# OliBomby/CM3P

Measured on AMD Instinct MI355X. Metric: contrastive training steps/sec (global beatmap-metadata pairs/sec), higher is better.
Workload: dtype bf16; 1 GPU; c2: default CM3P config, beatmap seq=4096, metadata seq=256, batch 32/GPU; global_batch=32, beatmap_seq=4096, metadata_seq=256, parallelism=dp1, weights=random init (reference init rules), fp32 master / bf16 GEMM operands

## Files before the change

cm3p_amd/_lib.py:

```python
from __future__ import annotations

import ctypes
import os
from ctypes import c_float, c_int, c_int64, c_uint64, c_void_p

import torch

F32, BF16 = 0, 1
ADD_A_BF16 = 16
POOL_PACKED = 2
GEMM_F32_TILED = 2
EPI_BF16, EPI_F32, EPI_F32_RESID, EPI_F32_BIAS, EPI_BF16_RESID = 0, 1, 2, 5, 7
EPI_BF16_GEGLU_FWD, EPI_BF16_GEGLU_BWD = 9, 10
ABI_VERSION = 20

_HERE = os.path.dirname(os.path.abspath(__file__))
LIB_PATH = os.environ.get("CM3P_HIP_LIB") or os.path.join(_HERE, "csrc", "libcm3p_hip.so")

_P, _I, _L, _F, _U64 = c_void_p, c_int, c_int64, c_float, c_uint64
_RETURNS_INT64 = {"cm3p_attn_bwd_fused_workspace_bytes", "cm3p_token_order_workspace_ints"}

SIGNATURES = {
    "cm3p_abi_version": [],
    "cm3p_layernorm_fwd": [_P, _I, _P, _P, _P, _P, _P, _L, _I, _F, _P],
    "cm3p_layernorm_bwd_blocks": [_L],
    "cm3p_layernorm_bwd": [_P, _I, _P, _I, _P, _P, _P, _P, _I, _P, _P, _P, _P, _L, _I, _P],
    "cm3p_embed_ln_fwd": [_P, _P, _I, _P, _P, _I, _P, _P, _P, _P, _P, _L, _I, _F, _L, _P],
    "cm3p_embed_ln_bwd": [_P, _I, _P, _P, _I, _P, _P, _I, _P, _P, _P, _P, _P, _P, _P, _L, _I, _L, _L, _P],
    "cm3p_embed_ln_bwd_sorted_chunk": [],
    "cm3p_embed_ln_bwd_sorted": [_P, _I, _P, _P, _P, _P, _I, _P, _P, _I, _P, _P, _P, _P, _P, _P, _P, _P, _P, _L, _I, _L, _L, _P],
    "cm3p_token_order_workspace_ints": [_L, _L],
    "cm3p_token_order": [_P, _L, _L, _P, _P, _P, _P],
    "cm3p_audio_slots": [_P, _L, _L, _P, _P, _P],
    "cm3p_gemm_bf16": [_P, _P, _P, _P, _L, _L, _L, _L, _L, _L, _I, _I, _I, _I, _P, _P],
    "cm3p_qkv_gemm_rope": [_P, _P, _P, _L, _L, _L, _P, _P, _I, _I, _I, _F, _P],
    "cm3p_gemm_wgrad_splits": [_L, _L, _L],
    "cm3p_gemm_route": [_L, _L, _L, _L, _L, _I, _I, _I, _I, _I, _I],
    "cm3p_gemm8p_set_grid": [_I],
    "cm3p_gemm8p_get_grid": [],
    "cm3p_build_ablation_flags": [],
    "cm3p_debug_set_dma_audit": [_P],
    "cm3p_cast_f32_bf16": [_P, _P, _L, _P],
    "cm3p_cast_f32_bf16_t": [_P, _P, _P, _L, _L, _P],
    "cm3p_cast_f32_bf16_t_multi": [_P, _I, _L, _P],
    "cm3p_add_f32": [_P, _P, _I, _P, _P, _L, _P],
    "cm3p_rope_table": [_P, _L, _P, _I, _P, _P, _P],
    "cm3p_rope_apply": [_P, _P, _P, _I, _I, _I, _L, _I, _P],
    "cm3p_attn_fwd": [_P, _P, _P, _P, _I, _I, _I, _I, _F, _I, _P],
    "cm3p_attn_fwd_impl": [_I, _I, _I, _I],
    "cm3p_attn_probs": [_P, _P, _P, _P, _I, _I, _I, _I, _F, _I, _P],
    "cm3p_attn_generic_supported": [_I],
    "cm3p_attn_fwd_generic": [_P, _P, _P, _P, _I, _I, _I, _I, _I, _F, _P],
    "cm3p_attn_bwd_generic": [_P, _P, _P, _P, _P, _P, _P, _I, _I, _I, _I, _I, _F, _P],
    "cm3p_attn_fwd_generic_dropout": [_P, _P, _P, _P, _I, _I, _I, _I, _I, _F, _I, _I, _U64, _P],
    "cm3p_attn_bwd_generic_dropout": [_P, _P, _P, _P, _P, _P, _P, _I, _I, _I, _I, _I, _F, _I, _I, _U64, _P],
    "cm3p_rope_apply_generic": [_P, _P, _P, _I, _I, _I, _I, _L, _I, _P],
    "cm3p_attn_bwd": [_P, _P, _P, _P, _P, _P, _P, _I, _I, _I, _I, _F, _P, _P, _L, _I, _I, _P],
    "cm3p_geglu_fwd": [_P, _P, _L, _I, _P],
    "cm3p_gemm_geglu": [_P, _P, _P, _L, _L, _L, _P],
    "cm3p_geglu_bwd": [_P, _P, _P, _L, _I, _P],
    "cm3p_dropout_f32": [_P, _P, _P, _P, _L, _I, _I, _P, _I, _I, _I, _I, _U64, _P],
    "cm3p_attn_fwd_dropout": [_P, _P, _P, _P, _I, _I, _I, _I, _F, _I, _I, _I, _U64, _P],
    "cm3p_attn_bwd_dropout": [_P, _P, _P, _P, _P, _P, _P, _I, _I, _I, _I, _F, _P, _P, _L, _I, _I, _I, _I, _U64, _P],
    "cm3p_attn_fwd_dropout_varlen": [_P, _P, _P, _P, _I, _I, _L, _I, _I, _F, _I, _I, _I, _U64, _P],
    "cm3p_attn_bwd_dropout_varlen": [_P, _P, _P, _P, _P, _P, _P, _I, _I, _L, _I, _I, _F, _P, _P, _I, _I, _I, _I, _U64, _P],
    "cm3p_geglu_fwd_dropout": [_P, _P, _L, _I, _I, _P, _I, _I, _I, _U64, _P],
    "cm3p_geglu_bwd_dropout": [_P, _P, _P, _L, _I, _I, _P, _I, _I, _I, _U64, _P],
    "cm3p_dropout_keep": [_P, _I, _I, _I, _I, _I, _I, _U64, _P],
    "cm3p_philox4x32_10_host": [_P, _P, _P, _L],
    "cm3p_gelu_fwd": [_P, _P, _L, _P],
    "cm3p_gelu_bwd": [_P, _P, _P, _L, _P],
    "cm3p_im2col_k3": [_P, _I, _P, _I, _I, _I, _I, _I, _P],
    "cm3p_col2im_k3": [_P, _P, _I, _I, _I, _I, _I, _P],
    "cm3p_bias_gelu_fwd": [_P, _P, _P, _P, _L, _I, _P],
    "cm3p_bias_gelu_bwd_blocks": [_L],
    "cm3p_bias_gelu_bwd": [_P, _I, _P, _P, _P, _P, _P, _L, _I, _P],
    "cm3p_pool_chunks": [_I],
    "cm3p_pool_fwd": [_P, _I, _P, _P, _P, _P, _I, _I, _I, _I, _P],
    "cm3p_pool_bwd": [_P, _P, _P, _P, _I, _I, _I, _I, _I, _P],
    "cm3p_gemm_f32": [_P, _P, _P, _I, _I, _I, _L, _L, _L, _L, _L, _F, _I, _P],
    "cm3p_l2norm_fwd": [_P, _P, _P, _I, _I, _P],
    "cm3p_l2norm_bwd": [_P, _P, _P, _P, _I, _I, _P],
    "cm3p_cross_entropy": [_P, _I, _I, _L, _L, _P, _P, _F, _P, _P, _P],
    "cm3p_cross_entropy_masked": [_P, _L, _I, _L, _P, _L, _F, _P, _P, _P, _P],
    "cm3p_inv_valid_count": [_P, _L, _L, _P, _P],
    "cm3p_ce_masked_stats": [_P, _L, _I, _L, _P, _L, _P, _P, _P],
    "cm3p_ce_masked_dlogits_blocks": [_L],
    "cm3p_ce_masked_dlogits_bf16": [_P, _L, _I, _L, _P, _L, _P, _P, _P, _P, _P, _P, _P],
    "cm3p_add_bias_f32": [_P, _P, _L, _I, _P],
    "cm3p_colsum_blocks": [_L],
    "cm3p_colsum_f32": [_P, _P, _P, _L, _I, _P],
    "cm3p_first_zero_index": [_P, _I, _I, _P, _P],
    "cm3p_scale_exp": [_P, _P, _P, _L, _P],
    "cm3p_scale_by": [_P, _P, _P, _L, _P],
    "cm3p_dot_f32": [_P, _P, _P, _L, _P],
    "cm3p_sum_f32": [_P, _P, _L, _F, _I, _P],
# ... 158 lines not shown
```

cm3p_amd/csrc/attention_bwd_fused.hip:

```cpp
#include <stdlib.h>

#include <type_traits>

#include "attn_common.h"

namespace {

#ifndef CM3P_FABL
#define CM3P_FABL 0
#endif

#ifndef CM3P_FTRACE
#define CM3P_FTRACE 0
#endif
#if CM3P_FTRACE
__device__ unsigned long long* g_bwdf_trace = nullptr;
#endif

constexpr int kFStage = 16384 + 512;
constexpr int kFSlots = 3;
constexpr int kFKimg = kFSlots * kFStage;
constexpr int kFdS = kFKimg + 32768;
constexpr int kFZ = kFdS + 2 * 32768;
constexpr int kFLds = kFZ + 4 * 2560;
constexpr int kFUnroll = 6;
constexpr int kFPadTiles = 12;

__host__ __device__ inline int64_t fused_stat_floats(int B, int S, int nh) { return (int64_t)B * nh * ((S + 63) / 64 + kFPadTiles) * 128; }
__host__ __device__ inline int fused_slab_rows(int S) { return ((S + 63) / 64) * 64 + 64; }
__host__ __device__ inline int fused_slabs(int S, int G = 2) { return ((S + 255) / 256 + G - 1) / G; }

__device__ __forceinline__ bf16x8 gload_frag8(const uint16_t* p) { return *reinterpret_cast<const bf16x8*>(p); }

__device__ __forceinline__ void mfma_av0(f32x16& d, const bf16x8& a, const bf16x8& b) {
    asm volatile("v_mfma_f32_32x32x16_bf16 %0, %1, %2, 0" : "=&v"(d) : "a"(a), "v"(b));
}
__device__ __forceinline__ void mfma_ava(f32x16& d, const bf16x8& a, const bf16x8& b) {
    asm volatile("v_mfma_f32_32x32x16_bf16 %0, %1, %2, %0" : "+v"(d) : "a"(a), "v"(b));
}
__device__ __forceinline__ void mfma_vva(f32x16& d, const bf16x8& a, const bf16x8& b) {
    asm volatile("v_mfma_f32_32x32x16_bf16 %0, %1, %2, %0" : "+v"(d) : "v"(a), "v"(b));
}

__device__ __forceinline__ void lds_barrier() {
    asm volatile("s_waitcnt lgkmcnt(0)" ::: "memory");
    __builtin_amdgcn_s_barrier();
    asm volatile("" ::: "memory");
}

template <bool PRE>
__device__ __forceinline__ void exp2c_pair(f32x16& s, int i, float cm) {
    if constexpr ((CM3P_FABL & 64) != 0) return;
    s[i] = __builtin_amdgcn_fmed3f(__builtin_amdgcn_exp2f(PRE ? s[i] : s[i] * cm), 0.f, 1.f);
    s[i + 1] = __builtin_amdgcn_fmed3f(__builtin_amdgcn_exp2f(PRE ? s[i + 1] : s[i + 1] * cm), 0.f, 1.f);
}

__global__ __launch_bounds__(256) void attn_bwd_prep_kernel(const uint16_t* __restrict__ o_rows, const uint16_t* __restrict__ d_o,
                                                            const float* __restrict__ lse, float* __restrict__ stat_ws, int Smax, int nh,
                                                            float lse_mul, VarLen vl) {
    const int t = blockIdx.x, head = blockIdx.y, b = blockIdx.z, tid = threadIdx.x;
    const SeqView sv(vl, b, head, Smax, nh);
    const int S = sv.S;
    const int row = t * 64 + (tid >> 2), part = tid & 3;
    const int64_t ldo = (int64_t)nh * 64;
    float acc = 0.f;
    if (row < S) {
        const uint16_t* po = o_rows + (sv.row0 + row) * ldo + head * 64 + part * 16;
        const uint16_t* pg = d_o + (sv.row0 + row) * ldo + head * 64 + part * 16;
#pragma unroll
        for (int h = 0; h < 2; ++h) {
            const bf16x8 a = gload_frag8(po + 8 * h), g = gload_frag8(pg + 8 * h);
#pragma unroll
            for (int j = 0; j < 8; ++j) acc += (float)a[j] * (float)g[j];
        }
    }
    acc += __shfl_xor(acc, 1, 64);
    acc += __shfl_xor(acc, 2, 64);
    if (part == 0) {
        float* st = stat_ws + (((int64_t)b * nh + head) * gridDim.x + t) * 128;
        const bool ok = row < S;
        st[tid >> 2] = ok ? lse[sv.stat0 + row] * lse_mul : kNegInf;
        st[64 + (tid >> 2)] = ok ? -acc : 0.f;
    }
}

__device__ __forceinline__ void dq_reduce_tile(const uint16_t* __restrict__ dq_part, uint16_t* __restrict__ dqkv, int t, int head, int b,
                                               int tid, const SeqView& sv, int Smax, int nh, float scale,
                                               const float* __restrict__ rope_cos, const float* __restrict__ rope_sin,
                                               int64_t pos_batch_stride, int G) {
    const int S = sv.S;
    const int row = t * 64 + (tid >> 2), j = tid & 3;
    if (row >= S) return;
    const int nkb = fused_slabs(Smax, G), nkb_b = fused_slabs(S, G);
    const int64_t slab = (int64_t)fused_slab_rows(Smax) * 64;
    const uint16_t* p = dq_part + ((int64_t)b * nh + head) * nkb * slab + (int64_t)row * 64 + 8 * j;
    float lo[8], hi[8];
#pragma unroll
    for (int i = 0; i < 8; ++i) lo[i] = hi[i] = 0.f;
    constexpr int kBatch = 8;
    for (int kb0 = 0; kb0 < nkb_b; kb0 += kBatch) {
        uint4 a[kBatch], c[kBatch];
#pragma unroll
        for (int u = 0; u < kBatch; ++u) {
            const int kb = min(kb0 + u, nkb_b - 1);
            a[u] = gload16<(CM3P_NT & 8) != 0>(p + kb * slab);
            c[u] = gload16<(CM3P_NT & 8) != 0>(p + kb * slab + 32);
        }
#pragma unroll
        for (int u = 0; u < kBatch; ++u) {
            if (kb0 + u < nkb_b) {
                lo[0] += bf16lo(a[u].x), lo[1] += bf16hi(a[u].x), lo[2] += bf16lo(a[u].y), lo[3] += bf16hi(a[u].y);
                lo[4] += bf16lo(a[u].z), lo[5] += bf16hi(a[u].z), lo[6] += bf16lo(a[u].w), lo[7] += bf16hi(a[u].w);
                hi[0] += bf16lo(c[u].x), hi[1] += bf16hi(c[u].x), hi[2] += bf16lo(c[u].y), hi[3] += bf16hi(c[u].y);
                hi[4] += bf16lo(c[u].z), hi[5] += bf16hi(c[u].z), hi[6] += bf16lo(c[u].w), hi[7] += bf16hi(c[u].w);
            }
        }
    }
    if (rope_cos) {
        const int64_t prow = sv.pos0(b, pos_batch_stride) + row;
#pragma unroll
        for (int h = 0; h < 2; ++h) {
            f32x4 lo4 = {lo[4 * h], lo[4 * h + 1], lo[4 * h + 2], lo[4 * h + 3]};
            f32x4 hi4 = {hi[4 * h], hi[4 * h + 1], hi[4 * h + 2], hi[4 * h + 3]};
            rope_rotate4<true>(lo4, hi4, rope_cos + prow * 32, rope_sin + prow * 32, 8 * j + 4 * h);
#pragma unroll
            for (int r = 0; r < 4; ++r) {
                lo[4 * h + r] = lo4[r];
                hi[4 * h + r] = hi4[r];
            }
        }
    }
    uint16_t* drow = dqkv + (sv.row0 + row) * ((int64_t)3 * nh * 64) + head * 64 + 8 * j;
    gstore16<(CM3P_NT & 8) != 0>(drow, uint4{pack_bf16x2(lo[0] * scale, lo[1] * scale), pack_bf16x2(lo[2] * scale, lo[3] * scale),
                                             pack_bf16x2(lo[4] * scale, lo[5] * scale), pack_bf16x2(lo[6] * scale, lo[7] * scale)});
    gstore16<(CM3P_NT & 8) != 0>(drow + 32, uint4{pack_bf16x2(hi[0] * scale, hi[1] * scale), pack_bf16x2(hi[2] * scale, hi[3] * scale),
                                                  pack_bf16x2(hi[4] * scale, hi[5] * scale), pack_bf16x2(hi[6] * scale, hi[7] * scale)});
}

__global__ __launch_bounds__(256) void attn_bwd_dq_reduce_kernel(const uint16_t* __restrict__ dq_part, uint16_t* __restrict__ dqkv, int Smax,
                                                                 int nh, float scale, const float* __restrict__ rope_cos,
                                                                 const float* __restrict__ rope_sin, int64_t pos_batch_stride, VarLen vl, int G) {
    const int head = blockIdx.y, b = blockIdx.z;
    const SeqView sv(vl, b, head, Smax, nh);
    dq_reduce_tile(dq_part, dqkv, blockIdx.x, head, b, threadIdx.x, sv, Smax, nh, scale, rope_cos, rope_sin, pos_batch_stride, G);
}

template <bool PRE, bool ADD>
__global__ __launch_bounds__(256, 1) void attn_bwd_fused_kernel(const uint16_t* __restrict__ qkv, const uint16_t* __restrict__ d_o,
                                                                const float* __restrict__ stat_ws, uint16_t* __restrict__ dq_part,
                                                                uint16_t* __restrict__ dqkv, const uint8_t* __restrict__ kmask, int Smax,
                                                                int nh, float scale, const float* __restrict__ rope_cos,
                                                                const float* __restrict__ rope_sin, int64_t pos_batch_stride, VarLen vl, int G,
                                                                int phase) {
    extern __shared__ __attribute__((aligned(16))) char smem[];
    const int tid = threadIdx.x, lane = tid & 63, hh = lane >> 5;
    const int wid = __builtin_amdgcn_readfirstlane(tid >> 6);
    const int nkb = (Smax + 255) / 256, NT = (Smax + 63) / 64;
    const int nblk = (nkb - phase + G - 1) / G;
    int kblk, head, b;
    decode_block(nblk, nh, kblk, head, b);
    const int slab_idx = kblk;
    kblk = G * kblk + phase;
    const int K0 = kblk * 256;
    const SeqView sv(vl, b, head, Smax, nh);
    const int S = sv.S;
// ... 419 lines not shown
            loadG_one(smem, sp, db, 0);
            loadG_one(smem, sp, db, 1);
        }
    mfma_vc(sA, Qf[0], kf[0][0], isv);
    mfma_vc(dpA, Gf[0], vf[0][0], idv);
#pragma unroll
    for (int s4 = 1; s4 < 4; ++s4) {
        mfma_va(sA, Qf[s4], kf[0][s4]);
        mfma_va(dpA, Gf[s4], vf[0][s4]);
    }
#pragma unroll
    for (int i = 0; i < 16; ++i) dq[i] = 0.f;
    load_dq_operand(dqB0, 1, 8);
    asm volatile("s_nop 15\n\ts_nop 15" ::: "memory");
    CM3P_SB();

#if CM3P_FTRACE
    const unsigned long long ft0 = __builtin_amdgcn_s_memtime();
#endif
    for (int t = 0; t < n_tiles + 2; t += kFUnroll) {
        tile(std::integral_constant<int, 0>{}, I0{}, t);
        tile(std::integral_constant<int, 1>{}, I1{}, t + 1);
        tile(std::integral_constant<int, 2>{}, I0{}, t + 2);
        tile(std::integral_constant<int, 0>{}, I1{}, t + 3);
        tile(std::integral_constant<int, 1>{}, I0{}, t + 4);
        tile(std::integral_constant<int, 2>{}, I1{}, t + 5);
    }
    asm volatile("s_waitcnt vmcnt(0)" ::: "memory");
#if CM3P_FTRACE
    if (g_bwdf_trace && lane == 0) {
        unsigned long long* o = g_bwdf_trace + (size_t)blockIdx.x * 16 + wid * 4;
        o[0] = ft_acc[0];
        o[1] = ft_acc[1];
        o[2] = __builtin_amdgcn_s_memtime() - ft0;
        o[3] = (unsigned long long)(n_tiles + 2 + kFUnroll - 1) / kFUnroll * kFUnroll;
    }
#endif


#pragma unroll
    for (int kb = 0; kb < 2; ++kb) {
        const int krow = k0 + 32 * kb + l31;
        if (krow < S) {
            const bool ok = kmask ? kmask[sv.row0 + krow] != 0 : true;
            const float ks = ok ? (PRE ? 0.69314718055994531f : scale) : 0.f, vs = ok ? 1.f : 0.f;
            uint16_t* dkrow = dqkv + (sv.row0 + krow) * ld + nh * 64 + head * 64;
            uint16_t* dvrow = dkrow + nh * 64;
            if (!ok) {
#pragma unroll
                for (int db = 0; db < 2; ++db)
#pragma unroll
                    for (int i = 0; i < 16; ++i) dk[db][kb][i] = dv[db][kb][i] = 0.f;
            }
            if (rope_cos) {
                const int64_t prow = sv.pos0(b, pos_batch_stride) + krow;
#pragma unroll
                for (int g = 0; g < 4; ++g) {
                    f32x4 lo4 = {dk[0][kb][4 * g], dk[0][kb][4 * g + 1], dk[0][kb][4 * g + 2], dk[0][kb][4 * g + 3]};
                    f32x4 hi4 = {dk[1][kb][4 * g], dk[1][kb][4 * g + 1], dk[1][kb][4 * g + 2], dk[1][kb][4 * g + 3]};
                    rope_rotate4<true>(lo4, hi4, rope_cos + prow * 32, rope_sin + prow * 32, 8 * g + 4 * hh);
#pragma unroll
                    for (int r = 0; r < 4; ++r) {
                        dk[0][kb][4 * g + r] = lo4[r];
                        dk[1][kb][4 * g + r] = hi4[r];
                    }
                }
            }
#pragma unroll
            for (int db = 0; db < 2; ++db)
#pragma unroll
                for (int g = 0; g < 4; ++g) {
                    const int d = 32 * db + 8 * g + 4 * hh;
                    *reinterpret_cast<uint2*>(dkrow + d) = uint2{pack_bf16x2(dk[db][kb][4 * g] * ks, dk[db][kb][4 * g + 1] * ks),
                                                                 pack_bf16x2(dk[db][kb][4 * g + 2] * ks, dk[db][kb][4 * g + 3] * ks)};
                    *reinterpret_cast<uint2*>(dvrow + d) = uint2{pack_bf16x2(dv[db][kb][4 * g] * vs, dv[db][kb][4 * g + 1] * vs),
                                                                 pack_bf16x2(dv[db][kb][4 * g + 2] * vs, dv[db][kb][4 * g + 3] * vs)};
                }
        }
    }
}

}

extern "C" {

int cm3p_attn_bwd_fused_slab_group(int S) {
    const char* e = getenv("CM3P_FUSED_SLAB_GROUP");
    if (e && (e[0] == '2' || e[0] == '4') && e[1] == '\0') return e[0] - '0';
    return (S + 255) / 256 >= 24 ? 4 : 2;
}

int64_t cm3p_attn_bwd_fused_workspace_bytes(int B, int S, int nh) {
    if (B <= 0 || S <= 0 || nh <= 0) return 0;
    const int64_t stats = (fused_stat_floats(B, S, nh) * 4 + 255) / 256 * 256;
    return stats + (int64_t)B * nh * fused_slabs(S) * fused_slab_rows(S) * 128;
}

int cm3p_attn_bwd_fused(const void* qkv, const void* out, const void* dout, const float* lse, void* dqkv, const uint8_t* key_mask,
                        const int* cu_seqlens, int B, int S, int64_t total, int nh, float scale, const float* cos_tab,
                        const float* sin_tab, int64_t pos_batch_stride, int stages, int q_prescaled, void* workspace,
                        int64_t workspace_bytes, void* stream) {
    CM3P_REQUIRE((cos_tab == nullptr) == (sin_tab == nullptr));
    CM3P_REQUIRE(stages >= 1 && stages <= 255);
    CM3P_REQUIRE(qkv && out && dout && lse && dqkv && workspace && B > 0 && S > 0 && nh > 0 && scale > 0.f);
    CM3P_REQUIRE(cm3p_aligned16(qkv) && cm3p_aligned16(out) && cm3p_aligned16(dout) && cm3p_aligned16(dqkv) && cm3p_aligned16(workspace));
    if (cu_seqlens) CM3P_REQUIRE(total > 0 && key_mask == nullptr && pos_batch_stride == 0);
    else CM3P_REQUIRE(pos_batch_stride == 0 || pos_batch_stride == S);
    CM3P_REQUIRE(workspace_bytes >= cm3p_attn_bwd_fused_workspace_bytes(B, S, nh));
    CM3P_REQUIRE((int64_t)S * 3 * nh * 128 < (int64_t)1 << 31);
    hipStream_t s = static_cast<hipStream_t>(stream);
    const VarLen vl{cu_seqlens, cu_seqlens ? total : 0};
    float* stat_ws = static_cast<float*>(workspace);
    uint16_t* dq_part = reinterpret_cast<uint16_t*>(static_cast<char*>(workspace) + (fused_stat_floats(B, S, nh) * 4 + 255) / 256 * 256);
    const int NT = (S + 63) / 64;
    const bool pre = q_prescaled != 0;
    const int G = cm3p_attn_bwd_fused_slab_group(S);
    CM3P_REQUIRE((stages & (7 * CM3P_ATTN_BWD_FUSED_MAIN_ADD1) & ~(((1 << (G - 1)) - 1) * CM3P_ATTN_BWD_FUSED_MAIN_ADD1)) == 0);
    if (stages & CM3P_ATTN_BWD_FUSED_PREP) {
        const float lse_mul = pre ? -kLog2e : -1.0f / scale;
        attn_bwd_prep_kernel<<<dim3(NT + kFPadTiles, nh, B), 256, 0, s>>>((const uint16_t*)out, (const uint16_t*)dout, lse, stat_ws, S, nh,
                                                                          lse_mul, vl);
        if (hipGetLastError() != hipSuccess) return CM3P_ERR_LAUNCH;
    }
    const bool run_even = stages & (CM3P_ATTN_BWD_FUSED_MAIN | CM3P_ATTN_BWD_FUSED_MAIN_EVEN);
    const bool run_odd = stages & (CM3P_ATTN_BWD_FUSED_MAIN | CM3P_ATTN_BWD_FUSED_MAIN_ODD);
    if (run_even || run_odd || (stages & (7 * CM3P_ATTN_BWD_FUSED_MAIN_ADD1))) {
        static Cm3pDevOnce once;
        const int rc_once = once.run([] {
            return cm3p_set_max_lds({reinterpret_cast<const void*>(&attn_bwd_fused_kernel<true, false>), reinterpret_cast<const void*>(&attn_bwd_fused_kernel<true, true>),
                                     reinterpret_cast<const void*>(&attn_bwd_fused_kernel<false, false>), reinterpret_cast<const void*>(&attn_bwd_fused_kernel<false, true>)},
                                    kFLds);
        });
        if (rc_once != CM3P_OK) return rc_once;
        const int nkb = (S + 255) / 256;
#define CM3P_FUSED_ARGS (const uint16_t*)qkv, (const uint16_t*)dout, stat_ws, dq_part, (uint16_t*)dqkv, key_mask, S, nh, scale, cos_tab, sin_tab, pos_batch_stride, vl, G
        if (run_even) {
            const dim3 grid0(((nkb + G - 1) / G) * nh * B);
            if (pre) attn_bwd_fused_kernel<true, false><<<grid0, 256, kFLds, s>>>(CM3P_FUSED_ARGS, 0);
            else attn_bwd_fused_kernel<false, false><<<grid0, 256, kFLds, s>>>(CM3P_FUSED_ARGS, 0);
            if (hipGetLastError() != hipSuccess) return CM3P_ERR_LAUNCH;
        }
        for (int phase = 1; phase < G && phase < nkb; ++phase) {
            if (!(run_odd || (stages & (CM3P_ATTN_BWD_FUSED_MAIN_ADD1 << (phase - 1))))) continue;
            const dim3 gridp(((nkb - phase + G - 1) / G) * nh * B);
            if (pre) attn_bwd_fused_kernel<true, true><<<gridp, 256, kFLds, s>>>(CM3P_FUSED_ARGS, phase);
            else attn_bwd_fused_kernel<false, true><<<gridp, 256, kFLds, s>>>(CM3P_FUSED_ARGS, phase);
            if (hipGetLastError() != hipSuccess) return CM3P_ERR_LAUNCH;
        }
#undef CM3P_FUSED_ARGS
    }
    if (stages & CM3P_ATTN_BWD_FUSED_REDUCE) {
        attn_bwd_dq_reduce_kernel<<<dim3(NT, nh, B), 256, 0, s>>>(dq_part, (uint16_t*)dqkv, S, nh, scale, cos_tab, sin_tab, pos_batch_stride, vl, G);
    }
    CM3P_LAUNCH_CHECK();
    return CM3P_OK;
}

}

int cm3p_ablation_flags_attention_bwd_fused() { return (CM3P_FABL) | ((CM3P_FTRACE) << 12); }
#if CM3P_FTRACE
extern "C" int cm3p_debug_set_bwdf_trace(unsigned long long* p) {
    return hipMemcpyToSymbol(HIP_SYMBOL(g_bwdf_trace), &p, sizeof(p)) == hipSuccess ? 0 : 1;
}
#endif

#if CM3P_DMA_AUDIT
int cm3p_audit_set_attention_bwd_fused(void* buf) { return cm3p_audit_set_local(buf); }
#endif
```

cm3p_amd/csrc/attn_common.h:

```cpp
#pragma once
#include <limits.h>

#include "common.h"

namespace {

constexpr float kLog2e = 1.4426950408889634f;
constexpr float kNegInf = -__builtin_huge_valf();

__device__ __forceinline__ int swz(int row) { return (((row >> 1) & 1) << 2) | ((row >> 2) & 3); }
__device__ __forceinline__ int off_R(int row, int c16) { return row * 128 + ((c16 ^ swz(row)) << 4); }
__device__ __forceinline__ int off_T(int row, int col) { return row * 128 + (((col >> 3) ^ swz(row)) << 4) + ((col & 7) << 1); }

__device__ __forceinline__ int xcd_remap(int n, int total) {
    const int q8 = total / 8, r8 = total % 8, xcd = n % 8;
    return (xcd < r8 ? xcd * (q8 + 1) : r8 * (q8 + 1) + (xcd - r8) * q8) + n / 8;
}
__device__ __forceinline__ void decode_block(int nblk, int nh, int& blk, int& head, int& b) {
    const int logical = xcd_remap(blockIdx.x, gridDim.x);
    blk = logical % nblk;
    const int bh = logical / nblk;
    head = bh % nh;
    b = bh / nh;
}

#ifndef CM3P_BAND_ORDER
#define CM3P_BAND_ORDER 1
#endif
__device__ __forceinline__ void decode_block_band(int nblk, int nh, int& blk, int& head, int& b) {
    if constexpr (CM3P_BAND_ORDER == 0) {
        decode_block(nblk, nh, blk, head, b);
    } else {
        const int logical = xcd_remap(blockIdx.x, gridDim.x);
        head = logical % nh;
        const int rb = logical / nh;
        blk = rb % nblk;
        b = rb / nblk;
    }
}

struct VarLen {
    const int* cu;
    int64_t total;
};
struct SeqView {
    int64_t row0;
    int64_t stat0;
    int S;
    bool packed;
    __device__ __forceinline__ SeqView(const VarLen& vl, int b, int head, int Smax, int nh) {
        packed = vl.cu != nullptr;
        if (packed) {
            row0 = vl.cu[b];
            S = vl.cu[b + 1] - vl.cu[b];
            stat0 = (int64_t)head * vl.total + row0;
        } else {
            row0 = (int64_t)b * Smax;
            S = Smax;
            stat0 = ((int64_t)b * nh + head) * Smax;
        }
    }
    __device__ __forceinline__ int64_t pos0(int b, int64_t pos_batch_stride) const { return packed ? row0 : (int64_t)b * pos_batch_stride; }
};

__device__ __forceinline__ f32x16 mfma32(bf16x8 a, bf16x8 b, f32x16 c) {
    return __builtin_amdgcn_mfma_f32_32x32x16_bf16(a, b, c, 0, 0, 0);
}

__device__ __forceinline__ bf16x8 frag_T(const char* tile, int krow0, int cblk, int lane) {
    const int g = lane >> 4, hh = g >> 1, i = lane & 15;
    const int row = krow0 + 4 * hh + (i >> 2);
    const int col = 32 * cblk + 16 * (g & 1) + 4 * (i & 3);
    const bf16x4 lo = lds_read_tr16(tile + off_T(row, col));
    const bf16x4 hi = lds_read_tr16(tile + off_T(row + 8, col));
    return cat_bf16x4(lo, hi);
}

__device__ __forceinline__ bf16x8 frag_R(const char* tile, int row0, int s, int lane) {
    return *reinterpret_cast<const bf16x8*>(tile + off_R(row0 + (lane & 31), 2 * s + (lane >> 5)));
}

__device__ __forceinline__ bf16x8 acc_to_frag(const f32x16& a, int sp) {
    bf16x8 r;
#pragma unroll
    for (int j = 0; j < 8; ++j) r[j] = (__bf16)a[8 * sp + j];
    return r;
}

__device__ __forceinline__ bf16x8 scale_frag(bf16x8 v, float c) {
    bf16x8 r;
#pragma unroll
    for (int j = 0; j < 8; ++j) r[j] = (__bf16)((float)v[j] * c);
    return r;
}

__device__ __forceinline__ float max3(float a, float b, float c) { return fmaxf(fmaxf(a, b), c); }

struct TileRegs64 {
    uint4 v[2];
};

__device__ __forceinline__ void gload64(TileRegs64& t, const uint16_t* base, int64_t ld, int r0, int limit, int tid) {
#pragma unroll
    for (int i = 0; i < 2; ++i) {
        const int q = tid + 256 * i, row = q >> 3, c = q & 7;
        const int r = r0 + row;
        t.v[i] = (r < limit && r >= 0) ? *reinterpret_cast<const uint4*>(base + (int64_t)r * ld + c * 8) : uint4{0u, 0u, 0u, 0u};
    }
}
__device__ __forceinline__ void lstore64_R(char* tile, const TileRegs64& t, int tid) {
#pragma unroll
    for (int i = 0; i < 2; ++i) {
        const int q = tid + 256 * i, row = q >> 3, c = q & 7;
        *reinterpret_cast<uint4*>(tile + off_R(row, c)) = t.v[i];
    }
}


#define CM3P_SB() __builtin_amdgcn_sched_barrier(0)

__device__ __forceinline__ void mfma_vc(f32x16& d, const bf16x8& a, const bf16x8& b, const f32x16& c) {
    asm volatile("v_mfma_f32_32x32x16_bf16 %0, %1, %2, %3" : "=&v"(d) : "v"(a), "a"(b), "v"(c));
}
__device__ __forceinline__ void mfma_va(f32x16& d, const bf16x8& a, const bf16x8& b) {
    asm volatile("v_mfma_f32_32x32x16_bf16 %0, %1, %2, %0" : "+v"(d) : "v"(a), "a"(b));
}
__device__ __forceinline__ bf16x8 ld_frag(const char* p) { return *reinterpret_cast<const bf16x8*>(p); }
__device__ __forceinline__ bf16x8 ld_fragT(const char* lo, const char* hi) { return cat_bf16x4(lds_read_tr16(lo), lds_read_tr16(hi)); }


__device__ __forceinline__ void store_rows32(char* buf, const f32x16& b0, const f32x16& b1, float mul, uint16_t* dst_row0, int64_t ld_elems,
                                             int nrows_valid, int lane) {
    const int l31 = lane & 31, hh = lane >> 5;
#pragma unroll
    for (int g = 0; g < 4; ++g) {
        *reinterpret_cast<uint2*>(buf + l31 * 144 + (8 * g + 4 * hh) * 2) =
            uint2{pack_bf16x2(b0[4 * g] * mul, b0[4 * g + 1] * mul), pack_bf16x2(b0[4 * g + 2] * mul, b0[4 * g + 3] * mul)};
        *reinterpret_cast<uint2*>(buf + l31 * 144 + (32 + 8 * g + 4 * hh) * 2) =
            uint2{pack_bf16x2(b1[4 * g] * mul, b1[4 * g + 1] * mul), pack_bf16x2(b1[4 * g + 2] * mul, b1[4 * g + 3] * mul)};
    }
    asm volatile("" ::: "memory");
#pragma unroll
    for (int i = 0; i < 4; ++i) {
        const int row = (lane >> 3) + 8 * i;
        const uint4 v = *reinterpret_cast<const uint4*>(buf + row * 144 + (lane & 7) * 16);
        if (row < nrows_valid) gstore16<(CM3P_NT & 4) != 0>(dst_row0 + row * ld_elems + (lane & 7) * 8, v);
    }
// ... 51 lines not shown
```

cm3p_amd/csrc/common.h:

```cpp
#pragma once
#include <hip/hip_runtime.h>
#include <stdint.h>

#include <atomic>
#include <initializer_list>
#include <mutex>
#include <type_traits>

#include "../../include/cm3p_hip.h"

typedef __attribute__((ext_vector_type(8))) __bf16 bf16x8;
typedef __attribute__((ext_vector_type(4))) __bf16 bf16x4;
typedef __attribute__((ext_vector_type(2))) __bf16 bf16x2;
typedef __attribute__((ext_vector_type(4))) float f32x4;
typedef __attribute__((ext_vector_type(8))) float f32x8;
typedef __attribute__((ext_vector_type(16))) float f32x16;

#define CM3P_WAVE 64
#define CM3P_EPI_BF16_ROPE 3
#define CM3P_EPI_BF16_AXPBY 4
#define CM3P_EPI_BF16_GEGLU 6

struct BatchArgs {
    int64_t a_stride = 0, b_stride = 0, c_stride = 0, r_stride = 0;
    const uint16_t* Rb = nullptr;
    float alpha = 1.f, beta = 0.f;
    void* C2 = nullptr;
};

#ifndef CM3P_NT
#define CM3P_NT 7
#endif
typedef __attribute__((ext_vector_type(4))) uint32_t cm3p_u32x4;
typedef __attribute__((ext_vector_type(2))) uint32_t cm3p_u32x2;
template <bool NT>
__device__ __forceinline__ void gstore16(void* p, cm3p_u32x4 v) {
    if constexpr (NT) __builtin_nontemporal_store(v, static_cast<cm3p_u32x4*>(p));
    else *static_cast<cm3p_u32x4*>(p) = v;
}
template <bool NT>
__device__ __forceinline__ void gstore16(void* p, uint4 v) { gstore16<NT>(p, cm3p_u32x4{v.x, v.y, v.z, v.w}); }
template <bool NT>
__device__ __forceinline__ void gstore16f(void* p, __attribute__((ext_vector_type(4))) float v) {
    gstore16<NT>(p, __builtin_bit_cast(cm3p_u32x4, v));
}
template <bool NT>
__device__ __forceinline__ void gstore8(void* p, uint2 v) {
    if constexpr (NT) __builtin_nontemporal_store(cm3p_u32x2{v.x, v.y}, static_cast<cm3p_u32x2*>(p));
    else *static_cast<uint2*>(p) = v;
}
template <bool NT>
__device__ __forceinline__ uint4 gload16(const void* p) {
    if constexpr (NT) {
        const cm3p_u32x4 v = __builtin_nontemporal_load(static_cast<const cm3p_u32x4*>(p));
        return uint4{v[0], v[1], v[2], v[3]};
    } else {
        return *static_cast<const uint4*>(p);
    }
}

template <bool NT>
__device__ __forceinline__ uint2 gload8(const void* p) {
    if constexpr (NT) {
        const cm3p_u32x2 v = __builtin_nontemporal_load(static_cast<const cm3p_u32x2*>(p));
        return uint2{v[0], v[1]};
    } else {
        return *static_cast<const uint2*>(p);
    }
}
template <bool NT>
__device__ __forceinline__ __attribute__((ext_vector_type(4))) float gload16f(const void* p) {
    typedef __attribute__((ext_vector_type(4))) float f4;
    if constexpr (NT) return __builtin_nontemporal_load(static_cast<const f4*>(p));
    else return *static_cast<const f4*>(p);
}

#ifndef CM3P_DMA_AUDIT
#define CM3P_DMA_AUDIT 0
#endif
enum { CM3P_AUD_A = 0, CM3P_AUD_B = 1, CM3P_AUD_T0 = 2, CM3P_AUD_T1 = 3, CM3P_AUD_S0 = 4, CM3P_AUD_S1 = 5, CM3P_AUD_SLOTS = 8 };
#if CM3P_DMA_AUDIT
static __device__ unsigned long long* cm3p_audit_buf = nullptr;
static inline int cm3p_audit_set_local(void* buf) {
    return hipMemcpyToSymbol(HIP_SYMBOL(cm3p_audit_buf), &buf, sizeof(buf)) == hipSuccess ? CM3P_OK : CM3P_ERR_LAUNCH;
}
__device__ __forceinline__ void cm3p_audit(int id, const void* first_byte, int bytes) {
    unsigned long long* buf = cm3p_audit_buf;
    if (!buf) return;
    unsigned long long lo = (unsigned long long)(uintptr_t)first_byte, hi = lo + (unsigned long long)bytes - 1ull;
#pragma unroll
    for (int o = 32; o > 0; o >>= 1) {
        const unsigned long long l2 = __shfl_xor(lo, o, 64), h2 = __shfl_xor(hi, o, 64);
        lo = l2 < lo ? l2 : lo;
        hi = h2 > hi ? h2 : hi;
    }
    if ((threadIdx.x & 63) == 0) {
        atomicMin(buf + 2 * id, lo);
        atomicMax(buf + 2 * id + 1, hi);
    }
}
#define CM3P_AUDIT(id, addr, bytes) cm3p_audit((id), (addr), (bytes))
#else
#define CM3P_AUDIT(id, addr, bytes) ((void)0)
#endif

#define CM3P_LAUNCH_CHECK()                                         \
    do {                                                            \
        hipError_t e__ = hipGetLastError();                         \
        if (e__ != hipSuccess) return CM3P_ERR_LAUNCH;              \
    } while (0)

// ... 90 lines not shown
    bf16x2 v = {(__bf16)lo, (__bf16)hi};
    return __builtin_bit_cast(uint32_t, v);
}
__device__ __forceinline__ float bf16lo(uint32_t w) { return __builtin_bit_cast(float, w << 16); }
__device__ __forceinline__ float bf16hi(uint32_t w) { return __builtin_bit_cast(float, w & 0xffff0000u); }
__device__ __forceinline__ uint32_t add_bf16x2(uint32_t a, uint32_t b) { return pack_bf16x2(bf16lo(a) + bf16lo(b), bf16hi(a) + bf16hi(b)); }

__device__ __forceinline__ void unpack8(const uint4 w, float (&f)[8]) {
    f[0] = bf16lo(w.x); f[1] = bf16hi(w.x); f[2] = bf16lo(w.y); f[3] = bf16hi(w.y);
    f[4] = bf16lo(w.z); f[5] = bf16hi(w.z); f[6] = bf16lo(w.w); f[7] = bf16hi(w.w);
}
__device__ __forceinline__ uint4 pack8(const float (&f)[8]) {
    return uint4{pack_bf16x2(f[0], f[1]), pack_bf16x2(f[2], f[3]), pack_bf16x2(f[4], f[5]), pack_bf16x2(f[6], f[7])};
}
__device__ __forceinline__ void geglu_bwd_item_f(const uint4 ha, const uint4 hb, const float (&d)[8], uint4& oa, uint4& ob) {
    float a[8], b[8], da[8], db[8];
    unpack8(ha, a);
    unpack8(hb, b);
#pragma unroll
    for (int j = 0; j < 8; j += 2) {
        const f32x2 av = {a[j], a[j + 1]};
        f32x2 cdf, pdf;
        gelu_cdf_pdf2(av, cdf, pdf);
        const f32x2 gr = av * pdf + cdf, gl = av * cdf;
        da[j] = d[j] * b[j] * gr.x;
        da[j + 1] = d[j + 1] * b[j + 1] * gr.y;
        db[j] = d[j] * gl.x;
        db[j + 1] = d[j + 1] * gl.y;
    }
    oa = pack8(da);
    ob = pack8(db);
}

struct RopeArgs {
    const float* cos;
    const float* sin;
    int S;
    int per_batch;
    int ncols;
    int q_cols = 0;
    float q_scale = 1.f;
};

enum { CM3P_GEMM_128 = 0, CM3P_GEMM_256 = 1, CM3P_GEMM_RING = 2 };
struct GemmRoute {
    int kernel;
    bool rebal;
    int splits;
    int64_t kchunk;
};
struct GemmCall {
    const void* A;
    const void* B;
    void* C;
    const float* R;
    int64_t M, N, K, lda, ldb, ldc;
    int a_kc, b_kc, epi;
    int64_t c_split_stride = 0;
    RopeArgs rope = RopeArgs{};
    BatchArgs bt = BatchArgs{};
    int batch = 0;
};
template <class F>
int cm3p_with_flag(bool v, F&& f) {
    return v ? f(std::true_type{}) : f(std::false_type{});
}
template <class F>
int cm3p_with_layout(bool a_kc, bool b_kc, F&& f) {
    return cm3p_with_flag(a_kc, [&](auto ak) { return cm3p_with_flag(b_kc, [&](auto bk) { return f(ak, bk); }); });
}
template <class F>
int cm3p_with_epilogue(int epi, F&& f) {
    switch (epi) {
        case CM3P_EPI_BF16: return f(std::integral_constant<int, CM3P_EPI_BF16>{});
        case CM3P_EPI_F32: return f(std::integral_constant<int, CM3P_EPI_F32>{});
        case CM3P_EPI_F32_RESID: return f(std::integral_constant<int, CM3P_EPI_F32_RESID>{});
        case CM3P_EPI_BF16_ROPE: return f(std::integral_constant<int, CM3P_EPI_BF16_ROPE>{});
        case CM3P_EPI_BF16_AXPBY: return f(std::integral_constant<int, CM3P_EPI_BF16_AXPBY>{});
        case CM3P_EPI_F32_BIAS: return f(std::integral_constant<int, CM3P_EPI_F32_BIAS>{});
        case CM3P_EPI_BF16_GEGLU: return f(std::integral_constant<int, CM3P_EPI_BF16_GEGLU>{});
        case CM3P_EPI_BF16_RESID: return f(std::integral_constant<int, CM3P_EPI_BF16_RESID>{});
        case CM3P_EPI_BF16_GEGLU_FWD: return f(std::integral_constant<int, CM3P_EPI_BF16_GEGLU_FWD>{});
        case CM3P_EPI_BF16_GEGLU_BWD: return f(std::integral_constant<int, CM3P_EPI_BF16_GEGLU_BWD>{});
        default: return CM3P_ERR_INTERNAL;
    }
}
constexpr bool cm3p_epi_is_geglu(int epi) {
    return epi == CM3P_EPI_BF16_GEGLU || epi == CM3P_EPI_BF16_GEGLU_FWD || epi == CM3P_EPI_BF16_GEGLU_BWD;
}
constexpr bool cm3p_gemm_pair_exists(bool a_kc, bool b_kc, int epi) {
    return (epi != CM3P_EPI_BF16_ROPE && epi != CM3P_EPI_F32_BIAS && !cm3p_epi_is_geglu(epi)) || (a_kc && b_kc);
}

template <bool INVERSE>
__device__ __forceinline__ void rope_rotate4(f32x4& a, f32x4& b, const float* cos_row, const float* sin_row, int d) {
    const f32x4 cs = *reinterpret_cast<const f32x4*>(cos_row + d);
    const f32x4 sn = *reinterpret_cast<const f32x4*>(sin_row + d);
    const f32x4 a0 = a, b0 = b;
    if constexpr (!INVERSE) {
        a = a0 * cs - b0 * sn;
        b = b0 * cs + a0 * sn;
    } else {
        a = a0 * cs + b0 * sn;
        b = b0 * cs - a0 * sn;
    }
}

__device__ __forceinline__ float wave_sum(float v) {
#pragma unroll
    for (int o = 32; o > 0; o >>= 1) v += __shfl_xor(v, o, 64);
    return v;
}
__device__ __forceinline__ float wave_max(float v) {
#pragma unroll
    for (int o = 32; o > 0; o >>= 1) v = fmaxf(v, __shfl_xor(v, o, 64));
    return v;
}

__device__ __forceinline__ bf16x4 lds_read_tr16(const void* p) {
    return __builtin_amdgcn_ds_read_tr16_b64_v4bf16((__attribute__((address_space(3))) bf16x4*)(p));
}

__device__ __forceinline__ bf16x8 cat_bf16x4(bf16x4 a, bf16x4 b) {
    return __builtin_shufflevector(a, b, 0, 1, 2, 3, 4, 5, 6, 7);
}
```

cm3p_amd/csrc/gemm.hip:

```cpp
#include <stdlib.h>

#include "common.h"

namespace {

constexpr int BM = 128, BN = 128, BK = 64;
constexpr int kStageBytes = BM * BK * 2;

__device__ __forceinline__ int kc_off(int r, int c) { return r * 128 + ((c ^ (r & 7)) << 4); }
__device__ __forceinline__ int ks_off(int k, int idx) {
    const int f = (k & 3) | (((k >> 3) & 1) << 2);
    return k * 256 + ((((idx >> 4) ^ f) & 7) << 5) + ((idx & 15) << 1);
}

template <bool KC>
struct TileLoader {
    const uint16_t* ptr[4];
    bool row_ok[4];
    int koff[4];
    int lds[4];
    int64_t kstep;

    __device__ __forceinline__ void init(const uint16_t* base, int64_t ld, int64_t idx0, int64_t extent, int64_t kbeg, int tid) {
#pragma unroll
// ... 90 lines not shown
        const char* sb = sa + kStageBytes;
        const bool more = kt + 1 < nk;
        if (more) {
            la.load(ra, kbeg + (int64_t)(kt + 1) * BK, kend);
            lb.load(rb, kbeg + (int64_t)(kt + 1) * BK, kend);
        }
#pragma unroll
        for (int kk = 0; kk < 2; ++kk) {
            bf16x8 fa[4], fb[4];
#pragma unroll
            for (int i = 0; i < 4; ++i) fa[i] = load_frag<A_KC>(sa, wm * 64 + i * 16, kk, lane);
#pragma unroll
            for (int j = 0; j < 4; ++j) fb[j] = load_frag<B_KC>(sb, wn * 64 + j * 16, kk, lane);
#pragma unroll
            for (int i = 0; i < 4; ++i)
#pragma unroll
                for (int j = 0; j < 4; ++j)
                    acc[i][j] = __builtin_amdgcn_mfma_f32_16x16x32_bf16(fb[j], fa[i], acc[i][j], 0, 0, 0);
        }
        if (more) {
            char* na = smem + ((kt + 1) & 1) * 2 * kStageBytes;
            la.store(na, ra);
            lb.store(na + kStageBytes, rb);
        }
        __syncthreads();
    }

#pragma unroll
    for (int i = 0; i < 4; ++i) {
        const int64_t m = m0 + wm * 64 + i * 16 + (lane & 15);
        if (m >= M) continue;
        if constexpr (EPI == CM3P_EPI_BF16_ROPE) {
            if (n0 + wn * 64 < rope.ncols) {
                const int64_t prow = rope.per_batch ? m : m % rope.S;
#pragma unroll
                for (int j = 0; j < 2; ++j)
                    rope_rotate4<false>(acc[i][j], acc[i][j + 2], rope.cos + prow * 32, rope.sin + prow * 32, j * 16 + 4 * (lane >> 4));
                if (n0 + wn * 64 < rope.q_cols) {
#pragma unroll
                    for (int j = 0; j < 4; ++j) acc[i][j] *= rope.q_scale;
                }
            }
        }
#pragma unroll
        for (int j = 0; j < 4; ++j) {
            const int64_t n = n0 + wn * 64 + j * 16 + 4 * (lane >> 4);
            if (n >= N) continue;
            f32x4 v = acc[i][j];
            if constexpr (EPI == CM3P_EPI_BF16 || EPI == CM3P_EPI_BF16_ROPE) {
                uint16_t* C = static_cast<uint16_t*>(Cv);
                *reinterpret_cast<uint2*>(C + m * ldc + n) = uint2{pack_bf16x2(v.x, v.y), pack_bf16x2(v.z, v.w)};
            } else if constexpr (EPI == CM3P_EPI_BF16_RESID) {
                uint16_t* C = static_cast<uint16_t*>(Cv);
                const uint2 r = *reinterpret_cast<const uint2*>(reinterpret_cast<const uint16_t*>(R) + m * ldc + n);
                *reinterpret_cast<uint2*>(C + m * ldc + n) = uint2{add_bf16x2(pack_bf16x2(v.x, v.y), r.x), add_bf16x2(pack_bf16x2(v.z, v.w), r.y)};
            } else if constexpr (EPI == CM3P_EPI_BF16_AXPBY) {
                uint16_t* C = static_cast<uint16_t*>(Cv) + (int64_t)blockIdx.y * bt.c_stride;
                v *= bt.alpha;
                if (bt.Rb) {
                    const uint2 r = *reinterpret_cast<const uint2*>(bt.Rb + (int64_t)blockIdx.y * bt.r_stride + m * ldc + n);
                    v += bt.beta * f32x4{bf16lo(r.x), bf16hi(r.x), bf16lo(r.y), bf16hi(r.y)};
                }
                *reinterpret_cast<uint2*>(C + m * ldc + n) = uint2{pack_bf16x2(v.x, v.y), pack_bf16x2(v.z, v.w)};
            } else {
                float* C = static_cast<float*>(Cv) + (int64_t)blockIdx.z * c_split_stride;
                if constexpr (EPI == CM3P_EPI_F32_RESID) v += *reinterpret_cast<const f32x4*>(R + m * ldc + n);
                if constexpr (EPI == CM3P_EPI_F32_BIAS) v += *reinterpret_cast<const f32x4*>(R + n);
                *reinterpret_cast<f32x4*>(C + m * ldc + n) = v;
            }
        }
    }
}

__global__ __launch_bounds__(256) void splitk_reduce_kernel(const float* __restrict__ ws, float* __restrict__ out, int64_t n4,
                                                            int splits, int64_t stride4) {
    for (int64_t i = (int64_t)blockIdx.x * 256 + threadIdx.x; i < n4; i += (int64_t)gridDim.x * 256) {
        f32x4 s = reinterpret_cast<const f32x4*>(ws)[i];
        for (int z = 1; z < splits; ++z) s += reinterpret_cast<const f32x4*>(ws)[i + z * stride4];
        reinterpret_cast<f32x4*>(out)[i] = s;
    }
}

template <bool A_KC, bool B_KC, int EPI>
constexpr bool has_instance = cm3p_gemm_pair_exists(A_KC, B_KC, EPI) && !cm3p_epi_is_geglu(EPI);

int launch128(const GemmRoute& r, const GemmCall& g, hipStream_t s) {
    const int tiles_m = (int)((g.M + BM - 1) / BM), tiles_n = (int)((g.N + BN - 1) / BN);
    const dim3 grid(tiles_m * tiles_n, g.batch > 0 ? g.batch : 1, r.splits);
    const size_t lds = 4 * kStageBytes;
    const uint16_t* a = static_cast<const uint16_t*>(g.A);
    const uint16_t* b = static_cast<const uint16_t*>(g.B);
    return cm3p_with_layout(g.a_kc, g.b_kc, [&](auto ak, auto bk) {
        return cm3p_with_epilogue(g.epi, [&](auto e) {
            constexpr bool AK = decltype(ak)::value, BK = decltype(bk)::value;
            constexpr int E = decltype(e)::value;
            if constexpr (has_instance<AK, BK, E>) {
                gemm_bf16_kernel<AK, BK, E><<<grid, 256, lds, s>>>(a, b, g.C, g.R, g.M, g.N, g.K, g.lda, g.ldb, g.ldc, tiles_n, r.kchunk,
                                                                 g.c_split_stride, g.rope, g.bt);
                return CM3P_OK;
            } else {
                return CM3P_ERR_INTERNAL;
            }
        });
    });
}

}

int cm3p_gemm256_dispatch(const GemmRoute& r, const GemmCall& g, hipStream_t s);
int cm3p_gemm8p_dispatch(const GemmRoute& r, const GemmCall& g, hipStream_t s);

static inline int64_t tiles_of(int64_t M, int64_t N, int t) { return ((M + t - 1) / t) * ((N + t - 1) / t); }
constexpr int64_t kBigItems = 200, kBigBatchItems = 128;

static GemmRoute cm3p_gemm_route_of(int64_t M, int64_t N, int64_t K, int64_t lda, int64_t ldb, bool a_kc, bool b_kc, int epi,
                                    int split_k, int rope_cols, int batch) {
    GemmRoute r{CM3P_GEMM_128, false, 1, K};
    const bool batched = epi == CM3P_EPI_BF16_AXPBY;
    if (M <= 0 || N <= 0 || K <= 0 || split_k < 1 || epi < 0 || epi > CM3P_EPI_BF16_GEGLU_BWD || epi == 8  || batched != (batch > 0) ||
        !cm3p_gemm_pair_exists(a_kc, b_kc, epi)) {
        r.kernel = CM3P_ERR_INVALID;
        return r;
    }
    const char* impl = getenv("CM3P_GEMM_IMPL");
    const bool no_ring = impl && impl[0] == '2', small_only = impl && impl[0] == '1';
    static const bool no_rebal = [] { const char* e = getenv("CM3P_G8P_REBAL"); return e && e[0] == '0'; }();
    if (split_k > 1) {
        const int64_t q = (K % 128 == 0) ? 128 : 64;
        r.kchunk = ((K + split_k - 1) / split_k + q - 1) / q * q;
        r.splits = (int)((K + r.kchunk - 1) / r.kchunk);
    }
    const int64_t items = tiles_of(M, N, 256) * (batched ? batch : r.splits);
    const bool ring_ok = M % 8 == 0 && N % 8 == 0 && lda * 16 < (int64_t(1) << 31) && ldb * 16 < (int64_t(1) << 31);
    bool big = K % 64 == 0 && r.kchunk % 64 == 0 && items >= (batched ? kBigBatchItems : kBigItems);
    if (epi == CM3P_EPI_BF16_GEGLU) {
        if (!(big && N % 64 == 0 && ring_ok)) r.kernel = CM3P_ERR_INVALID;
        else r.kernel = no_ring ? CM3P_GEMM_256 : CM3P_GEMM_RING;
    } else if (epi == CM3P_EPI_BF16_GEGLU_FWD || epi == CM3P_EPI_BF16_GEGLU_BWD) {
        const int64_t cols = epi == CM3P_EPI_BF16_GEGLU_FWD ? 64 : 32;
        r.kernel = (big && N % cols == 0 && ring_ok && split_k == 1 && !no_ring && !small_only) ? CM3P_GEMM_RING : CM3P_ERR_INVALID;
    } else if (batched) {
        const bool filled = M * N * batch * 10 >= items * 65536 * 7;
        big = big && filled && (a_kc || !b_kc) && ring_ok && !no_ring;
        if (big) r.kernel = CM3P_GEMM_RING;
    } else {
        big = big && !small_only;
        if (epi == CM3P_EPI_BF16_ROPE) big = big && rope_cols % 256 == 0 && M < (int64_t(1) << 31);
        if (big) r.kernel = (ring_ok && !no_ring) ? CM3P_GEMM_RING : CM3P_GEMM_256;
    }
    if (r.kernel > CM3P_GEMM_128) {
        const int64_t last = K - (int64_t)(r.splits - 1) * r.kchunk;
        r.rebal = !no_rebal && (r.kchunk / 64) % 2 == 0 && (last / 64) % 2 == 0;
    }
    return r;
}

static int run_routed(const GemmRoute& r, const GemmCall& g, hipStream_t s) {
    int rc = CM3P_ERR_INVALID;
    if (r.kernel == CM3P_GEMM_RING) rc = cm3p_gemm8p_dispatch(r, g, s);
    else if (r.kernel == CM3P_GEMM_256) rc = cm3p_gemm256_dispatch(r, g, s);
    else if (r.kernel == CM3P_GEMM_128) rc = launch128(r, g, s);
    if (rc != CM3P_OK) return rc;
    CM3P_LAUNCH_CHECK();
    return CM3P_OK;
}

int cm3p_ablation_flags_attention();
int cm3p_ablation_flags_attention_bwd_fused();
int cm3p_ablation_flags_gemm256();
int cm3p_ablation_flags_gemm8p();
int cm3p_ablation_flags_attention_fwd();
#if CM3P_DMA_AUDIT
int cm3p_audit_set_attention_fwd(void*);
int cm3p_audit_set_gemm8p(void*);
int cm3p_audit_set_gemm256(void*);
int cm3p_audit_set_attention(void*);
int cm3p_audit_set_attention_bwd_fused(void*);
#endif

extern "C" {

int cm3p_build_ablation_flags(void) {
    return (cm3p_ablation_flags_attention() != 0) | (cm3p_ablation_flags_attention_bwd_fused() != 0) << 2 |
           (cm3p_ablation_flags_gemm256() != 0) << 3 | (cm3p_ablation_flags_gemm8p() != 0) << 4 | (CM3P_DMA_AUDIT != 0) << 5 |
           (cm3p_ablation_flags_attention_fwd() != 0) << 6;
}

int cm3p_debug_set_dma_audit(void* buf) {
#if CM3P_DMA_AUDIT
    int rc = cm3p_audit_set_gemm8p(buf);
    if (rc == CM3P_OK) rc = cm3p_audit_set_gemm256(buf);
    if (rc == CM3P_OK) rc = cm3p_audit_set_attention(buf);
    if (rc == CM3P_OK) rc = cm3p_audit_set_attention_bwd_fused(buf);
    if (rc == CM3P_OK) rc = cm3p_audit_set_attention_fwd(buf);
    return rc;
#else
    (void)buf;
    return CM3P_ERR_INVALID;
#endif
}

int cm3p_gemm_wgrad_splits(int64_t M, int64_t N, int64_t K) {
    const int64_t t256 = tiles_of(M, N, 256);
    if (K % 64 == 0 && K >= 8192) {
        int64_t s = 256 / t256;
        if (s > K / 2048) s = K / 2048;
        if (s < 1) s = 1;
        if (t256 * s >= kBigItems) return (int)s;
    }
    const int64_t t128 = tiles_of(M, N, 128);
    if (t128 >= 512 || K <= 1024) return 1;
    int64_t s = (1024 + t128 - 1) / t128;
    if (s > K / 512) s = K / 512;
    return (int)(s < 1 ? 1 : s);
}

int cm3p_gemm_route(int64_t M, int64_t N, int64_t K, int64_t lda, int64_t ldb, int a_kc, int b_kc, int epilogue, int split_k,
                    int rope_cols, int batch) {
    const GemmRoute r = cm3p_gemm_route_of(M, N, K, lda, ldb, a_kc != 0, b_kc != 0, epilogue, split_k, rope_cols, batch);
    return r.kernel < 0 ? CM3P_ERR_INVALID : (r.kernel | (r.rebal ? 4 : 0) | r.splits << 3);
}

int cm3p_qkv_gemm_rope(const void* x, const void* Wqkv, void* qkv, int64_t M, int64_t N, int64_t K, const float* cos_tab,
                       const float* sin_tab, int S, int per_batch, int rope_cols, float q_scale, void* stream) {
    CM3P_REQUIRE(x && Wqkv && qkv && cos_tab && sin_tab && M > 0 && N > 0 && K > 0 && S > 0);
    CM3P_REQUIRE(cm3p_aligned16(x) && cm3p_aligned16(Wqkv) && cm3p_aligned16(qkv) && cm3p_aligned16(cos_tab) && cm3p_aligned16(sin_tab));
    CM3P_REQUIRE(K % 8 == 0 && N % 64 == 0 && rope_cols % 64 == 0 && rope_cols >= 0 && rope_cols <= N);
    CM3P_REQUIRE(per_batch || M % S == 0);
    CM3P_REQUIRE(q_scale > 0.f && rope_cols % 2 == 0);
    const GemmRoute r = cm3p_gemm_route_of(M, N, K, K, K, true, true, CM3P_EPI_BF16_ROPE, 1, rope_cols, 0);
    CM3P_REQUIRE(r.kernel >= 0);
    GemmCall g{x, Wqkv, qkv, nullptr, M, N, K, K, K, N, 1, 1, CM3P_EPI_BF16_ROPE};
    g.rope = RopeArgs{cos_tab, sin_tab, S, per_batch, rope_cols, rope_cols / 2, q_scale};
    return run_routed(r, g, static_cast<hipStream_t>(stream));
}

int cm3p_gemm_bf16(const void* A, const void* B, void* C, const float* R, int64_t M, int64_t N, int64_t K, int64_t lda,
                   int64_t ldb, int64_t ldc, int a_kc, int b_kc, int epilogue, int split_k, float* workspace, void* stream) {
    CM3P_REQUIRE(A && B && C && M > 0 && N > 0 && K > 0);
    const bool geglu_fwd = epilogue == CM3P_EPI_BF16_GEGLU_FWD, geglu_bwd = epilogue == CM3P_EPI_BF16_GEGLU_BWD;
    CM3P_REQUIRE((epilogue >= CM3P_EPI_BF16 && epilogue <= CM3P_EPI_F32_RESID) || epilogue == CM3P_EPI_F32_BIAS || epilogue == CM3P_EPI_BF16_RESID ||
                 geglu_fwd || geglu_bwd);
    CM3P_REQUIRE(cm3p_aligned16(A) && cm3p_aligned16(B) && cm3p_aligned16(C));
    CM3P_REQUIRE(lda % 8 == 0 && ldb % 8 == 0 && ldc % 4 == 0 && N % 4 == 0);
    CM3P_REQUIRE(a_kc ? (K % 8 == 0 && lda >= K) : (M % 8 == 0 && lda >= M));
    CM3P_REQUIRE(b_kc ? (K % 8 == 0 && ldb >= K) : (N % 8 == 0 && ldb >= N));
    CM3P_REQUIRE(ldc >= N);
    CM3P_REQUIRE((epilogue != CM3P_EPI_F32_RESID && epilogue != CM3P_EPI_F32_BIAS && epilogue != CM3P_EPI_BF16_RESID && !geglu_bwd) || (R && cm3p_aligned16(R)));
    CM3P_REQUIRE(!geglu_fwd || (workspace && cm3p_aligned16(workspace) && ldc == N && N % 64 == 0 && split_k == 1));
    CM3P_REQUIRE(!geglu_bwd || (ldc == 2 * N && N % 32 == 0 && split_k == 1));
    CM3P_REQUIRE(epilogue != CM3P_EPI_BF16_RESID || (N % 8 == 0 && ldc % 8 == 0));
    CM3P_REQUIRE(split_k >= 1 && (split_k == 1 || (epilogue == CM3P_EPI_F32 && workspace && cm3p_aligned16(workspace) && ldc == N)));
    const GemmRoute r = cm3p_gemm_route_of(M, N, K, lda, ldb, a_kc != 0, b_kc != 0, epilogue, split_k, 0, 0);
    CM3P_REQUIRE(r.kernel >= 0);
    hipStream_t s = static_cast<hipStream_t>(stream);
    GemmCall g{A, B, C, R, M, N, K, lda, ldb, ldc, a_kc != 0, b_kc != 0, epilogue};
    if (geglu_fwd) g.bt.C2 = workspace;
    if (r.splits > 1) {
        g.C = workspace;
        g.c_split_stride = M * N;
    }
    const int rc = run_routed(r, g, s);
    if (rc != CM3P_OK) return rc;
    if (r.splits > 1) {
        const int64_t n4 = M * N / 4;
        int64_t blocks = (n4 + 255) / 256;
        if (blocks > 2048) blocks = 2048;
        splitk_reduce_kernel<<<(int)blocks, 256, 0, s>>>(workspace, static_cast<float*>(C), n4, r.splits, n4);
        CM3P_LAUNCH_CHECK();
    }
    return CM3P_OK;
}

int cm3p_gemm_geglu(const void* x, const void* w_interleaved, void* a, int64_t T, int64_t I, int64_t K, void* stream) {
    CM3P_REQUIRE(x && w_interleaved && a && T > 0 && I > 0 && K > 0);
    CM3P_REQUIRE(cm3p_aligned16(x) && cm3p_aligned16(w_interleaved) && cm3p_aligned16(a));
    GemmRoute r = cm3p_gemm_route_of(T, 2 * I, K, K, K, true, true, CM3P_EPI_BF16_GEGLU, 1, 0, 0);
    CM3P_REQUIRE(r.kernel >= 0);
    r.kernel = CM3P_GEMM_RING;
    const GemmCall g{x, w_interleaved, a, nullptr, T, 2 * I, K, K, K, I, 1, 1, CM3P_EPI_BF16_GEGLU};
    return run_routed(r, g, static_cast<hipStream_t>(stream));
}

int cm3p_gemm_bf16_batched(const void* A, const void* B, void* C, const void* R, int batch, int64_t M, int64_t N, int64_t K,
                           int64_t lda, int64_t ldb, int64_t ldc, int64_t stride_a, int64_t stride_b, int64_t stride_c,
                           int64_t stride_r, int a_kc, int b_kc, float alpha, float beta, void* stream) {
    CM3P_REQUIRE(A && B && C && batch > 0 && batch <= 65535 && M > 0 && N > 0 && K > 0);
    CM3P_REQUIRE(cm3p_aligned16(A) && cm3p_aligned16(B) && cm3p_aligned16(C) && (!R || cm3p_aligned16(R)));
    CM3P_REQUIRE(lda % 8 == 0 && ldb % 8 == 0 && ldc % 8 == 0 && N % 8 == 0 && ldc >= N);
    CM3P_REQUIRE(stride_a % 8 == 0 && stride_b % 8 == 0 && stride_c % 8 == 0 && stride_r % 8 == 0);
    CM3P_REQUIRE(a_kc ? (K % 8 == 0 && lda >= K) : (M % 8 == 0 && lda >= M));
    CM3P_REQUIRE(b_kc ? (K % 8 == 0 && ldb >= K) : (N % 8 == 0 && ldb >= N));
    const GemmRoute r = cm3p_gemm_route_of(M, N, K, lda, ldb, a_kc != 0, b_kc != 0, CM3P_EPI_BF16_AXPBY, 1, 0, batch);
    CM3P_REQUIRE(r.kernel >= 0);
    GemmCall g{A, B, C, nullptr, M, N, K, lda, ldb, ldc, a_kc != 0, b_kc != 0, CM3P_EPI_BF16_AXPBY};
    g.bt = BatchArgs{stride_a, stride_b, stride_c, stride_r, static_cast<const uint16_t*>(R), alpha, beta};
    g.batch = batch;
    return run_routed(r, g, static_cast<hipStream_t>(stream));
}

}
```

cm3p_amd/csrc/gemm256.hip:

```cpp
#include "common.h"

namespace {

constexpr int TM = 256, TN = 256, TK = 64;
#ifndef CM3P_G256_WN
#define CM3P_G256_WN 4
#endif
constexpr int kWN = CM3P_G256_WN;
constexpr int kThreads = 128 * kWN;
constexpr int kNJ = 16 / kWN;
constexpr int kWaveN = TN / kWN;
#ifndef CM3P_G256_ABL
#define CM3P_G256_ABL 0
#endif
constexpr int kPieces = 16 / kWN;
constexpr int kItems = 2048 / kThreads;
constexpr int kOperandBytes = TM * TK * 2;
constexpr int kStage = 2 * kOperandBytes;

__device__ __forceinline__ int kc_off(int r, int c) { return r * 128 + ((c ^ (r & 7)) << 4); }
__device__ __forceinline__ int ksf(int k) { return (k & 3) | (((k >> 3) & 1) << 2); }
__device__ __forceinline__ int ks_off(int k, int idx) { return k * 512 + (((idx >> 4) ^ ksf(k)) << 5) + ((idx & 15) << 1); }

__device__ __forceinline__ void glds16(const void* gsrc, char* lds_wave_base) {
// ... 250 lines not shown
                        if (m < M && n < N) {
                            uint4 x = *reinterpret_cast<const uint4*>(ebuf + r * kRow + ch * 16);
                            if constexpr (EPI == CM3P_EPI_BF16_RESID) {
                                const uint4 rb = *reinterpret_cast<const uint4*>(reinterpret_cast<const uint16_t*>(R) + m * ldc + n);
                                x = uint4{add_bf16x2(x.x, rb.x), add_bf16x2(x.y, rb.y), add_bf16x2(x.z, rb.z), add_bf16x2(x.w, rb.w)};
                            }
                            if constexpr (EPI == CM3P_EPI_BF16) {
                                if (n + 8 > N) {
                                    *reinterpret_cast<uint2*>(C + m * ldc + n) = uint2{x.x, x.y};
                                    continue;
                                }
                            }
                            *reinterpret_cast<uint4*>(C + m * ldc + n) = x;
                        }
                    }
                }
                lds_barrier();
            }
        } else {
            constexpr int kRow = TN * 4 + 16;
            float* C = static_cast<float*>(Cv) + (int64_t)z * c_split_stride;
            f32x4 rres[kItems];
            auto load_resid = [&](int pass) {
                if constexpr (EPI == CM3P_EPI_F32_RESID) {
#pragma unroll
                    for (int u = 0; u < kItems; ++u) {
                        const int id = tid + kThreads * u, r = id >> 6, ch = id & 63;
                        const int64_t m = m0 + pass * 32 + r, n = n0 + ch * 4;
                        rres[u] = (m < M && n < N) ? *reinterpret_cast<const f32x4*>(R + m * ldc + n) : f32x4{0.f, 0.f, 0.f, 0.f};
                    }
                }
                if constexpr (EPI == CM3P_EPI_F32_BIAS) {
                    if (pass == 0) {
#pragma unroll
                        for (int u = 0; u < kItems; ++u) {
                            const int64_t n = n0 + ((tid + kThreads * u) & 63) * 4;
                            rres[u] = n < N ? *reinterpret_cast<const f32x4*>(R + n) : f32x4{0.f, 0.f, 0.f, 0.f};
                        }
                    }
                }
            };
            load_resid(0);
#pragma unroll
            for (int pass = 0; pass < 8; ++pass) {
                if (wm == (pass >> 2)) {
#pragma unroll
                    for (int i2 = 0; i2 < 2; ++i2)
#pragma unroll
                        for (int j = 0; j < kNJ; ++j) {
                            const f32x4 a = acc[(pass & 3) * 2 + i2][j];
                            const int r = i2 * 16 + (lane & 15), cidx = wn * kWaveN + j * 16 + 4 * (lane >> 4);
                            *reinterpret_cast<f32x4*>(ebuf + r * kRow + cidx * 4) = a;
                        }
                }
                lds_barrier();
                f32x4 rcur[kItems];
#pragma unroll
                for (int u = 0; u < kItems; ++u) rcur[u] = rres[u];
                if (pass < 7) load_resid(pass + 1);
#pragma unroll
                for (int u = 0; u < kItems; ++u) {
                    const int id = tid + kThreads * u, r = id >> 6, ch = id & 63;
                    const int64_t m = m0 + pass * 32 + r, n = n0 + ch * 4;
                    if (m < M && n < N) {
                        f32x4 a = *reinterpret_cast<const f32x4*>(ebuf + r * kRow + ch * 16);
                        if constexpr (EPI == CM3P_EPI_F32_RESID || EPI == CM3P_EPI_F32_BIAS) a += rcur[u];
                        *reinterpret_cast<f32x4*>(C + m * ldc + n) = a;
                    }
                }
                lds_barrier();
            }
        }

        if (!has_next) break;
        v = vn;
        m0 = m0n;
        n0 = n0n;
        z = zn;
        nk = nkn;
    }
}

template <bool A_KC, bool B_KC, int EPI>
constexpr bool has_instance = cm3p_gemm_pair_exists(A_KC, B_KC, EPI) && !cm3p_epi_is_geglu(EPI) && EPI != CM3P_EPI_BF16_AXPBY;

}

int cm3p_gemm256_dispatch(const GemmRoute& r, const GemmCall& g, hipStream_t s) {
    const int tiles_m = (int)((g.M + TM - 1) / TM), tiles_n = (int)((g.N + TN - 1) / TN);
    const int ntiles = tiles_m * tiles_n, total = ntiles * r.splits;
    const int num_cu = cm3p_num_cu();
    const dim3 grid(total < num_cu ? total : num_cu);
    const size_t lds = 2 * kStage;
    const uint16_t* a = static_cast<const uint16_t*>(g.A);
    const uint16_t* b = static_cast<const uint16_t*>(g.B);
    return cm3p_with_layout(g.a_kc, g.b_kc, [&](auto ak, auto bk) {
        return cm3p_with_epilogue(g.epi, [&](auto e) {
            constexpr bool AK = decltype(ak)::value, BK = decltype(bk)::value;
            constexpr int E = decltype(e)::value;
            if constexpr (has_instance<AK, BK, E>) {
                static Cm3pDevOnce once;
                const int rc_once = once.run([&] { return cm3p_set_max_lds({(const void*)gemm256_kernel<AK, BK, E>}, (int)lds); });
                if (rc_once != CM3P_OK) return rc_once;
                gemm256_kernel<AK, BK, E><<<grid, kThreads, lds, s>>>(a, b, g.C, g.R, g.M, g.N, g.K, g.lda, g.ldb, g.ldc, tiles_n, ntiles, total,
                                                                    r.kchunk, g.c_split_stride, g.rope);
                return CM3P_OK;
            } else {
                return CM3P_ERR_INTERNAL;
            }
        });
    });
}

int cm3p_ablation_flags_gemm256() { return (CM3P_G256_ABL) | ((CM3P_G256_WN != 4) << 8); }
#if CM3P_DMA_AUDIT
int cm3p_audit_set_gemm256(void* buf) { return cm3p_audit_set_local(buf); }
#endif
```

cm3p_amd/csrc/gemm8p.hip:

```cpp
#include <stdlib.h>

#include <type_traits>

#include "common.h"

#ifndef CM3P_G8P_ABL
#define CM3P_G8P_ABL 0
#endif
#ifndef CM3P_G8P_DELAY
#define CM3P_G8P_DELAY 10
#endif

namespace {

constexpr int kHalf = 16384;
constexpr int kRing = 8 * kHalf;
constexpr int kEpiWave = 4096;
constexpr int kLds8p = kRing + 8 * kEpiWave;
enum { kAL = 0, kAH = 1, kBL = 2, kBH = 3 };
__host__ __device__ constexpr int slot_off(int par, int kind) { return (par * 4 + kind) * kHalf; }

template <int IMM, int AUD = CM3P_AUD_A>
__device__ __forceinline__ void glds_s(uint32_t voff, const char* sbase, uint32_t ldsw) {
    CM3P_AUDIT(AUD, sbase + voff, 16);
    if constexpr (CM3P_G8P_ABL & 64) {
        asm volatile("" ::"v"(voff), "s"(sbase), "s"(ldsw));
        return;
    }
    asm volatile("s_add_u32 m0, %2, %3\n\ts_nop 0\n\tglobal_load_lds_dwordx4 %0, %1" ::"v"(voff), "s"(sbase), "s"(ldsw), "n"(IMM)
                 : "memory", "m0", "scc");
}

typedef __attribute__((ext_vector_type(4))) uint32_t u32x4;


#if CM3P_G8P_ABL & 1
#define G8P_GLOBAL(stmt) asm volatile("" ::: "memory")
#else
#define G8P_GLOBAL(stmt) stmt
#endif
#define G8P_LANE_XCHG_FENCE() asm volatile("" ::: "memory")
#define G8P_WAIT_LGKM(n) asm volatile("s_waitcnt lgkmcnt(" #n ")" ::: "memory")
#define G8P_WAIT_VM(n) asm volatile("s_waitcnt vmcnt(" #n ")" ::: "memory")

template <bool KC, bool IS_A>
struct Operand {
    static constexpr int G = IS_A ? 64 : 32;
    const char* p[2][2];
    uint32_t voff[2];
    int64_t kstep;
    int fbase;

    __device__ __forceinline__ void init(int64_t ld, int wid, int lane) {
        const int wx = IS_A ? (wid >> 2) : (wid & 3);
        if constexpr (KC) {
            kstep = 128;
            voff[0] = voff[1] = (uint32_t)((lane >> 3) * (int)ld * 2 + (((lane & 7) ^ (lane >> 3)) << 4));
            fbase = (wx * G + (lane & 15)) * 128 + (((lane >> 4) ^ (lane & 7)) << 4);
        } else {
            kstep = 128 * ld;
            const int g = lane >> 4, q = (lane >> 2) & 3, pp = lane & 3;
            fbase = (8 * g + q) * 256 + 8 * pp + (((wx * (G / 16)) ^ (q | ((g & 1) << 2))) << 5);
        }
    }
    __device__ __forceinline__ void setup(const uint16_t* X, int64_t ld, int64_t idx0, int64_t extent, int64_t kbeg, int wid, int lane) {
        if constexpr (KC) {
#pragma unroll
            for (int h = 0; h < 2; ++h)
#pragma unroll
                for (int i = 0; i < 2; ++i) {
                    const int j = 16 * wid + 8 * i;
                    int64_t idx = idx0 + (j / G) * 2 * G + h * G + j % G;
                    if (idx > extent - 8) idx = extent - 8;
                    p[h][i] = reinterpret_cast<const char*>(X + idx * ld + kbeg);
                }
        } else {
#pragma unroll
            for (int i = 0; i < 2; ++i) p[0][i] = p[1][i] = reinterpret_cast<const char*>(X + (kbeg + 8 * wid + 4 * i) * ld + idx0);
            const int kl = lane >> 4, c = lane & 15;
            const int seg = (c >> 1) ^ (kl | ((wid & 1) << 2));
            const int j = seg * 16 + (c & 1) * 8;
#pragma unroll
            for (int h = 0; h < 2; ++h) {
                int64_t idx = idx0 + (j / G) * 2 * G + h * G + j % G;
                if (idx > extent - 8) idx = extent - 8;
                voff[h] = (uint32_t)(kl * (int)ld * 2 + (int)(idx - idx0) * 2);
// ... 334 lines not shown
#pragma unroll
                for (int j4 = 0; j4 < 4; ++j4) {
                    const f32x4 a = acc[i4][j4];
                    const int row = lane & 15, s8 = (j4 * 4 + (lane >> 4)) ^ ((row & 7) << 1);
                    *reinterpret_cast<uint2*>(eb + row * 128 + s8 * 8) = uint2{pack_bf16x2(a.x, a.y), pack_bf16x2(a.z, a.w)};
                }
                G8P_LANE_XCHG_FENCE();
                const int r0 = lane >> 3, r1 = 8 + (lane >> 3), ch = lane & 7;
                const int row = lane >> 2, dc = lane & 3;
                const u32x4 x0 = *reinterpret_cast<const u32x4*>(eb + r0 * 128 + ((ch ^ (r0 & 7)) << 4));
                const u32x4 x1 = *reinterpret_cast<const u32x4*>(eb + r1 * 128 + ((ch ^ (r1 & 7)) << 4));
                const u32x4 xh = *reinterpret_cast<const u32x4*>(eb + row * 128 + ((dc ^ (row & 7)) << 4));
                const u32x4 xg = *reinterpret_cast<const u32x4*>(eb + row * 128 + (((dc + 4) ^ (row & 7)) << 4));
                G8P_LANE_XCHG_FENCE();
                const bool col_ok = FULL || nw + ch * 8 < N;
                if (FULL || (col_ok && mw + i4 * 16 + r0 < M)) G8P_GLOBAL(gstore16<(CM3P_NT & 1) != 0>(Cb + (uint32_t)(i4 * 16 + r0) * ldcb + ch * 16, x0));
                if (FULL || (col_ok && mw + i4 * 16 + r1 < M)) G8P_GLOBAL(gstore16<(CM3P_NT & 1) != 0>(Cb + (uint32_t)(i4 * 16 + r1) * ldcb + ch * 16, x1));
                u32x4 y;
#pragma unroll
                for (int t = 0; t < 4; ++t) {
                    const f32x2 gl = gelu_erf2(f32x2{bf16lo(xh[t]), bf16hi(xh[t])});
                    y[t] = pack_bf16x2(gl.x * bf16lo(xg[t]), gl.y * bf16hi(xg[t]));
                }
                if (FULL || (mw + i4 * 16 + row < M && nw + dc * 8 < N))
                    G8P_GLOBAL(gstore16<(CM3P_NT & 1) != 0>(Ab + (uint32_t)(i4 * 16 + row) * ldab + dc * 16, y));
                if constexpr (CM3P_G8P_ABL & 1) asm volatile("" ::"v"(x0), "v"(x1), "v"(y));
            }
        } else if constexpr (EPI == CM3P_EPI_BF16_GEGLU_BWD) {
            char* Cb = reinterpret_cast<char*>(static_cast<uint16_t*>(Cv) + mw * ldc + nw);
            const char* Hb = reinterpret_cast<const char*>(reinterpret_cast<const uint16_t*>(R) + mw * ldc + 2 * nw);
            const uint32_t ldcb = (uint32_t)ldc * 2, upb = (uint32_t)N * 2;
            const int r0 = lane >> 3, ch = lane & 7;
            const uint32_t hoff = (uint32_t)((ch >> 2) * 128 + (ch & 3) * 16);
            const bool col_ok = FULL || nw + ch * 8 < N;
            u32x4 ga0, up0, ga1, up1;
            auto load_h = [&](int i4) {
                const bool ok0 = FULL || (col_ok && mw + i4 * 16 + r0 < M), ok1 = FULL || (col_ok && mw + i4 * 16 + 8 + r0 < M);
                const char* p0 = Hb + (uint32_t)(i4 * 16 + r0) * ldcb + hoff;
                const char* p1 = Hb + (uint32_t)(i4 * 16 + 8 + r0) * ldcb + hoff;
                const u32x4 zero = {0u, 0u, 0u, 0u};
                if constexpr (CM3P_G8P_ABL & 1) {
                    asm volatile("" : "=v"(ga0), "=v"(up0), "=v"(ga1), "=v"(up1) : "v"(p0), "v"(p1));
                } else {
                    ga0 = ok0 ? __builtin_bit_cast(u32x4, gload16<(CM3P_NT & 64) != 0>(p0)) : zero;
                    up0 = ok0 ? __builtin_bit_cast(u32x4, gload16<(CM3P_NT & 64) != 0>(p0 + 64)) : zero;
                    ga1 = ok1 ? __builtin_bit_cast(u32x4, gload16<(CM3P_NT & 64) != 0>(p1)) : zero;
                    up1 = ok1 ? __builtin_bit_cast(u32x4, gload16<(CM3P_NT & 64) != 0>(p1 + 64)) : zero;
                }
            };
            load_h(0);
#pragma unroll
            for (int i4 = 0; i4 < 8; ++i4) {
                char* eb = ebuf + (i4 & 1) * 2048;
#pragma unroll
                for (int j4 = 0; j4 < 4; ++j4) {
                    const f32x4 a = acc[i4][j4];
                    const int row = lane & 15, s8 = (j4 * 4 + (lane >> 4)) ^ ((row & 7) << 1);
                    *reinterpret_cast<uint2*>(eb + row * 128 + s8 * 8) = uint2{pack_bf16x2(a.x, a.y), pack_bf16x2(a.z, a.w)};
                }
                G8P_LANE_XCHG_FENCE();
                const int r1 = 8 + r0;
                const u32x4 x0 = *reinterpret_cast<const u32x4*>(eb + r0 * 128 + ((ch ^ (r0 & 7)) << 4));
                const u32x4 x1 = *reinterpret_cast<const u32x4*>(eb + r1 * 128 + ((ch ^ (r1 & 7)) << 4));
                G8P_LANE_XCHG_FENCE();
                const u32x4 g0 = ga0, u0 = up0, g1 = ga1, u1 = up1;
                if (i4 < 7) load_h(i4 + 1);
                float d[8];
                uint4 oa, ob;
                unpack8(uint4{x0[0], x0[1], x0[2], x0[3]}, d);
                geglu_bwd_item_f(uint4{g0[0], g0[1], g0[2], g0[3]}, uint4{u0[0], u0[1], u0[2], u0[3]}, d, oa, ob);
                if (FULL || (col_ok && mw + i4 * 16 + r0 < M)) {
                    G8P_GLOBAL(gstore16<(CM3P_NT & 1) != 0>(Cb + (uint32_t)(i4 * 16 + r0) * ldcb + ch * 16, oa));
                    G8P_GLOBAL(gstore16<(CM3P_NT & 1) != 0>(Cb + (uint32_t)(i4 * 16 + r0) * ldcb + upb + ch * 16, ob));
                }
                if constexpr (CM3P_G8P_ABL & 1) asm volatile("" ::"v"(oa.x), "v"(ob.x));
                unpack8(uint4{x1[0], x1[1], x1[2], x1[3]}, d);
                geglu_bwd_item_f(uint4{g1[0], g1[1], g1[2], g1[3]}, uint4{u1[0], u1[1], u1[2], u1[3]}, d, oa, ob);
                if (FULL || (col_ok && mw + i4 * 16 + r1 < M)) {
                    G8P_GLOBAL(gstore16<(CM3P_NT & 1) != 0>(Cb + (uint32_t)(i4 * 16 + r1) * ldcb + ch * 16, oa));
                    G8P_GLOBAL(gstore16<(CM3P_NT & 1) != 0>(Cb + (uint32_t)(i4 * 16 + r1) * ldcb + upb + ch * 16, ob));
                }
                if constexpr (CM3P_G8P_ABL & 1) asm volatile("" ::"v"(oa.x), "v"(ob.x));
            }
        } else if constexpr (EPI == CM3P_EPI_BF16_AXPBY) {
            char* Cb = reinterpret_cast<char*>(static_cast<uint16_t*>(Cv) + (int64_t)z * bt.c_stride + mw * ldc + nw);
            const char* Rb = reinterpret_cast<const char*>(bt.Rb + (int64_t)z * bt.r_stride + mw * ldc + nw);
            const uint32_t ldcb = (uint32_t)ldc * 2;
            const int lrow = lane >> 4, lch = lane & 15;
            const uint32_t loff = (uint32_t)lrow * ldcb + lch * 8;
            const bool col_ok = FULL || nw + lch * 4 < N;
#pragma unroll
            for (int i4 = 0; i4 < 8; ++i4) {
                uint2 r[4];
                if (bt.Rb) {
#pragma unroll
                    for (int u = 0; u < 4; ++u) {
                        const int row = i4 * 16 + u * 4;
                        r[u] = (FULL || (col_ok && mw + row + lrow < M)) ? *reinterpret_cast<const uint2*>(Rb + loff + (uint32_t)row * ldcb) : uint2{0u, 0u};
                    }
                }
#pragma unroll
                for (int j4 = 0; j4 < 4; ++j4) {
                    const int row = lane & 15, ch = j4 * 4 + (lane >> 4);
                    *reinterpret_cast<f32x4*>(ebuf + row * 256 + ((ch ^ row) << 4)) = acc[i4][j4];
                }
                G8P_LANE_XCHG_FENCE();
                f32x4 x[4];
#pragma unroll
                for (int u = 0; u < 4; ++u) {
                    const int row = u * 4 + lrow;
                    x[u] = *reinterpret_cast<const f32x4*>(ebuf + row * 256 + ((lch ^ row) << 4));
                }
                G8P_LANE_XCHG_FENCE();
#pragma unroll
                for (int u = 0; u < 4; ++u) {
                    f32x4 v = x[u];
                    v *= bt.alpha;
                    if (bt.Rb) v += bt.beta * f32x4{bf16lo(r[u].x), bf16hi(r[u].x), bf16lo(r[u].y), bf16hi(r[u].y)};
                    const int row = i4 * 16 + u * 4;
                    if (FULL || (col_ok && mw + row + lrow < M))
                        G8P_GLOBAL(*reinterpret_cast<uint2*>(Cb + loff + (uint32_t)row * ldcb) = (uint2{pack_bf16x2(v.x, v.y), pack_bf16x2(v.z, v.w)}));
                    if constexpr (CM3P_G8P_ABL & 1) asm volatile("" ::"v"(v));
                }
            }
        } else {
            char* Cb = reinterpret_cast<char*>(static_cast<float*>(Cv) + (int64_t)z * c_split_stride + mw * ldc + nw);
            const char* Rb = reinterpret_cast<const char*>(R + mw * ldc + nw);
            const uint32_t ldcb = (uint32_t)ldc * 4;
            const int lrow = lane >> 4, lch = lane & 15;
            const uint32_t loff = (uint32_t)lrow * ldcb + lch * 16;
            const bool col_ok = FULL || nw + lch * 4 < N;
            f32x4 rnext[4];
            auto load_r = [&](int i4) {
                if constexpr (EPI == CM3P_EPI_F32_RESID && !(CM3P_G8P_ABL & 1)) {
#pragma unroll
                    for (int u = 0; u < 4; ++u) {
                        const int row = i4 * 16 + u * 4;
                        rnext[u] = (FULL || (col_ok && mw + row + lrow < M)) ? gload16f<(CM3P_NT & 64) != 0>(Rb + loff + (uint32_t)row * ldcb)
                                                                             : f32x4{0.f, 0.f, 0.f, 0.f};
                    }
                }
            };
            f32x4 bias = f32x4{0.f, 0.f, 0.f, 0.f};
            if constexpr (EPI == CM3P_EPI_F32_BIAS) {
                if (col_ok) bias = *reinterpret_cast<const f32x4*>(R + nw + lch * 4);
            }
            load_r(0);
#pragma unroll
            for (int i4 = 0; i4 < 8; ++i4) {
#pragma unroll
                for (int j4 = 0; j4 < 4; ++j4) {
                    const int row = lane & 15, ch = j4 * 4 + (lane >> 4);
                    *reinterpret_cast<f32x4*>(ebuf + row * 256 + ((ch ^ row) << 4)) = acc[i4][j4];
                }
                G8P_LANE_XCHG_FENCE();
                f32x4 x[4];
#pragma unroll
                for (int u = 0; u < 4; ++u) {
                    const int row = u * 4 + lrow;
                    x[u] = *reinterpret_cast<const f32x4*>(ebuf + row * 256 + ((lch ^ row) << 4));
                }
                G8P_LANE_XCHG_FENCE();
#pragma unroll
                for (int u = 0; u < 4; ++u) {
                    if constexpr (EPI == CM3P_EPI_F32_RESID && !(CM3P_G8P_ABL & 1)) x[u] += rnext[u];
                    if constexpr (EPI == CM3P_EPI_F32_BIAS) x[u] += bias;
// ... 104 lines not shown
```

cm3p_amd/encoder.py:

```python
from __future__ import annotations

import os
import weakref
from typing import Optional

import torch
from torch import nn

from . import kernels as K

Tensor = torch.Tensor


def _check_supported(cfg):
    H, nh = cfg.hidden_size, cfg.num_attention_heads
    problems = []
    if H % nh or H // nh not in (16, 32, 64, 96, 128):
        problems.append(f"head_dim must be 64 (or 16 / 32 on the generic kernels, or 96 / 128 on the wide-head MFMA kernels); hidden_size={H}, heads={nh}")
    if getattr(cfg, "hidden_activation", "gelu") != "gelu":
        problems.append("hidden_activation must be 'gelu'")
    for flag in ("norm_bias", "attention_bias", "mlp_bias"):
        if getattr(cfg, flag, False):
            problems.append(f"{flag}=True is not supported (the reference configs never set it)")
    for p in ("attention_dropout", "embedding_dropout", "mlp_dropout"):
# ... 74 lines not shown


def _bf16_weight_pair(w: Tensor, want_t: bool):
    if not want_t:
        return _bf16_weight_cached(w), None
    w = w.detach()
    if w.dtype == torch.float32 and w.dim() == 2 and w.shape[0] % 8 == 0 and w.shape[1] % 8 == 0:
        return K.cast_bf16_with_transpose(w.contiguous())
    return _bf16_weight(w), None


class _Geometry:

    __slots__ = ("B", "S", "H", "I", "nh", "L", "eps", "windows", "key_mask", "rope", "per_batch_pos", "save", "cu", "max_s", "checkpoint",
                 "handoff", "attn_out", "wcast", "hd", "drop", "bf16", "fused_mlp")


def _hand_upstream(geo: _Geometry, gx32: Tensor, gx16: Optional[Tensor]) -> None:
    geo.handoff = (gx32, gx16)


def _take_from_downstream(geo: _Geometry, dy: Tensor):
    h, geo.handoff = geo.handoff, None
    if h is not None and h[1] is not None and h[0].data_ptr() == dy.data_ptr() and h[0].shape == dy.shape and dy.dtype == torch.float32 \
            and dy.is_contiguous():
        return h[0], h[1]
    g = dy.float().contiguous()
    if g.data_ptr() == dy.data_ptr():
        g = g.clone()
    return g, K.cast_bf16(g)


def _take_bf16_from_downstream(geo: _Geometry, dy: Tensor) -> Tensor:
    h, geo.handoff = geo.handoff, None
    if h is not None and h[0].data_ptr() == dy.data_ptr() and h[0].shape == dy.shape and dy.dtype == torch.bfloat16 and dy.is_contiguous():
        return h[0]
    g = dy.to(torch.bfloat16).contiguous()
    if g.data_ptr() == dy.data_ptr():
        g = g.clone()
    return g


def _layer_forward(geo: _Geometry, i: int, x: Tensor, wb, want_stats: bool):
    w_an, Wqkv_b, Wo_b, w_mn, Wi_b, Wo2_b = wb[:6]
    B, S, nh = geo.B, geo.S, geo.nh
    scale = geo.hd ** -0.5
    cos, sin = geo.rope[i]
    ad = (geo.drop.attn, geo.drop.seed, i) if geo.drop is not None and geo.drop.attn else None
    if i == 0:
        xn, mean_a, rstd_a = (x if x.dtype == torch.bfloat16 else K.cast_bf16(x)), None, None
    else:
        _, xn, mean_a, rstd_a = K.layernorm_fwd(x, w_an, geo.eps, False, True, want_stats)
    if geo.hd != 64:
        qkv = K.linear_fwd(xn, Wqkv_b)
        K.rope_apply_generic_(qkv, cos, sin, B, S, nh, geo.hd, geo.per_batch_pos)
        o, lse = K.attn_fwd_generic(qkv, geo.key_mask, B, S, nh, geo.hd, geo.windows[i], scale, drop=ad)
    elif geo.cu is not None:
        qkv = K.qkv_linear_rope(xn, Wqkv_b, cos, sin, S, geo.per_batch_pos, q_scale=K.SOFTMAX_Q_SCALE)
        o, lse = K.attn_fwd_varlen(qkv, geo.cu, B, geo.max_s, nh, geo.windows[i], scale, prescaled=True, drop=ad)
    else:
        qkv = K.qkv_linear_rope(xn, Wqkv_b, cos, sin, S, geo.per_batch_pos, q_scale=K.SOFTMAX_Q_SCALE)
        o, lse = K.attn_fwd(qkv, geo.key_mask, B, S, nh, geo.windows[i], scale, prescaled=True, drop=ad)
        if geo.attn_out is not None and len(geo.attn_out) == i:
            geo.attn_out.append(K.attn_probs(qkv, lse, geo.key_mask, B, S, nh, geo.windows[i], scale, prescaled=True))
    if ad is not None:
        x_mid = K.dropout_f32(K.linear_fwd_f32(o, Wo_b), ad[0], ad[1], i, K.SITE_ATTN_OUT, geo.S, geo.cu, resid=x)
    else:
        x_mid = K.linear_fwd(o, Wo_b, resid=x)
    _, xn2, mean_m, rstd_m = K.layernorm_fwd(x_mid, w_mn, geo.eps, False, True, want_stats)
    if len(wb) > 6 and wb[6] is not None:
        h, g = None, K.gemm_geglu(xn2, wb[6])
    elif len(wb) > 7 and wb[7]:
        h, g = K.linear_geglu_fwd(xn2, Wi_b)
    else:
        h = K.linear_fwd(xn2, Wi_b)
        if geo.drop is not None and geo.drop.mlp:
            g = K.geglu_fwd_dropout(h, geo.drop.mlp, geo.drop.seed, i, geo.S, geo.cu)
        else:
            g = K.geglu_fwd(h)
    x_out = K.linear_fwd(g, Wo2_b, resid=x_mid)
    return x_out, (x, xn, mean_a, rstd_a, qkv, o, lse, x_mid, xn2, mean_m, rstd_m, h, g)


def _attn_backward(geo: _Geometry, i: int, qkv: Tensor, o: Tensor, do: Tensor, lse: Tensor, ad: Optional[tuple]) -> Tensor:
    B, S, nh, window, scale = geo.B, geo.S, geo.nh, geo.windows[i], geo.hd ** -0.5
    if geo.hd != 64:
        dqkv = K.attn_bwd_generic(qkv, o, do, lse, geo.key_mask, B, S, nh, geo.hd, window, scale, drop=ad)
        return K.rope_apply_generic_(dqkv, geo.rope[i][0], geo.rope[i][1], B, S, nh, geo.hd, geo.per_batch_pos, inverse=True)
    if geo.cu is not None:
        return K.attn_bwd_varlen(qkv, o, do, lse, geo.cu, B, geo.max_s, nh, window, scale, geo.rope[i], prescaled=True, drop=ad)
    return K.attn_bwd(qkv, o, do, lse, geo.key_mask, B, S, nh, window, scale, geo.rope[i], geo.per_batch_pos, prescaled=True, drop=ad)


class _EncoderLayerFn(torch.autograd.Function):

    @staticmethod
    def forward(ctx, geo: _Geometry, i: int, x: Tensor, *weights: Tensor):
        it = iter(weights)
        w_an = None if i == 0 else _f32(next(it))
        Wqkv, Wo, w_mn, Wi, Wo2 = next(it), next(it), _f32(next(it)), next(it), next(it)
        fuse_geglu = (not geo.save) and not (geo.drop is not None and geo.drop.mlp) and Wi.dim() == 2 and K.gemm_geglu_supported(x.shape[0], Wi.shape[0] // 2, Wi.shape[1]) \
            and os.environ.get("CM3P_GEGLU_FUSED", "1") != "0"
        pre = geo.wcast if geo.save and geo.wcast is not None else {}
        pairs = [pre.get(id(w)) or _bf16_weight_pair(w, geo.save) if not (fuse_geglu and w is Wi) else (None, None) for w in (Wqkv, Wo, Wi, Wo2)]
        fused_train = geo.save and id(Wi) in geo.fused_mlp
        wb = (w_an, pairs[0][0], pairs[1][0], w_mn, pairs[2][0], pairs[3][0], _bf16_weight_cached(Wi, True) if fuse_geglu else None, fused_train)
        x_out, acts = _layer_forward(geo, i, x, wb, geo.save)
        if geo.save:
            ctx.saved = (x,) if geo.checkpoint else acts
            ctx.geo, ctx.i, ctx.wb = geo, i, wb
            ctx.wt = tuple(p[1] for p in pairs)
            ctx.wdtypes = [w.dtype for w in weights]
        return x_out

    @staticmethod
    def _backward_bf16(ctx, dy: Tensor):
        geo, i = ctx.geo, ctx.i
        need = ctx.needs_input_grad
        need_w = list(need[3:])
        if i == 0:
            need_w.insert(0, False)
        n_an, n_qkv, n_o, n_mn, n_i, n_o2 = need_w
        g = _take_bf16_from_downstream(geo, dy)
        if geo.checkpoint:
            _, acts = _layer_forward(geo, i, ctx.saved[0], ctx.wb, True)
        else:
            acts = ctx.saved
        x, xn, mean_a, rstd_a, qkv, o, lse, x_mid, xn2, mean_m, rstd_m, h, ga = acts
        del acts
        ctx_wb = ctx.wb
        w_an, Wqkv_b, Wo_b, w_mn, Wi_b, Wo2_b = ctx_wb[:6]
        Wqkv_t, Wo_t, Wi_t, Wo2_t = ctx.wt
        ctx.saved = ctx.wb = ctx.wt = None
        fused = len(ctx_wb) > 7 and ctx_wb[7]
        dg = None if fused else K.linear_dgrad(g, Wo2_b, Wo2_t)
        dWo2 = K.linear_wgrad(g, ga) if n_o2 else None
        dh = K.linear_dgrad_geglu_bwd(g, Wo2_t, h) if fused else K.geglu_bwd(dg, h)
        del dg, ga
        dxn2 = K.linear_dgrad(dh, Wi_b, Wi_t)
        dWi = K.linear_wgrad(dh, xn2) if n_i else None
        del dh, h, xn2
        _, g, dw_mn = K.layernorm_bwd(dxn2, x_mid, w_mn, mean_m, rstd_m, g, False, bf16_only=True)
        del dxn2, x_mid
        do = K.linear_dgrad(g, Wo_b, Wo_t)
        dWo = K.linear_wgrad(g, o) if n_o else None
        dqkv = _attn_backward(geo, i, qkv, o, do, lse, None)
        del do, o, qkv
        dWqkv = K.linear_wgrad(dqkv, xn) if n_qkv else None
        dw_an = None
        if i == 0:
            if need[2]:
                _, g = K.add_f32(g, K.linear_dgrad(dqkv, Wqkv_b, Wqkv_t))
            _hand_upstream(geo, g, g)
        elif need[2] or n_an:
            dxn = K.linear_dgrad(dqkv, Wqkv_b, Wqkv_t)
            _, g, dw_an = K.layernorm_bwd(dxn, x, w_an, mean_a, rstd_a, g, False, bf16_only=True)
            _hand_upstream(geo, g, g)
        grads = [dWqkv, dWo, dw_mn, dWi, dWo2] if i == 0 else [dw_an, dWqkv, dWo, dw_mn, dWi, dWo2]
        out = [(gw if gw.dtype == dt else gw.to(dt)) if (nd and gw is not None) else None for gw, dt, nd in zip(grads, ctx.wdtypes, need[3:])]
        return (None, None, g if need[2] else None, *out)

    @staticmethod
    def backward(ctx, dy: Tensor):
        if ctx.geo.bf16:
            return _EncoderLayerFn._backward_bf16(ctx, dy)
        geo, i = ctx.geo, ctx.i
        need = ctx.needs_input_grad
        need_w = list(need[3:])
        if i == 0:
            need_w.insert(0, False)
        n_an, n_qkv, n_o, n_mn, n_i, n_o2 = need_w
        gx32, gx16 = _take_from_downstream(geo, dy)
        if geo.checkpoint:
            _, acts = _layer_forward(geo, i, ctx.saved[0], ctx.wb, True)
        else:
            acts = ctx.saved
        x, xn, mean_a, rstd_a, qkv, o, lse, x_mid, xn2, mean_m, rstd_m, h, g = acts
        del acts
        ctx_wb = ctx.wb
        w_an, Wqkv_b, Wo_b, w_mn, Wi_b, Wo2_b = ctx_wb[:6]
        Wqkv_t, Wo_t, Wi_t, Wo2_t = ctx.wt
        ctx.saved = ctx.wb = ctx.wt = None
        fused = len(ctx_wb) > 7 and ctx_wb[7]
        dg = None if fused else K.linear_dgrad(gx16, Wo2_b, Wo2_t)
        dWo2 = K.linear_wgrad(gx16, g) if n_o2 else None
        if fused:
            dh = K.linear_dgrad_geglu_bwd(gx16, Wo2_t, h)
        elif geo.drop is not None and geo.drop.mlp:
            dh = K.geglu_bwd_dropout(dg, h, geo.drop.mlp, geo.drop.seed, i, geo.S, geo.cu)
        else:
            dh = K.geglu_bwd(dg, h)
        del dg, g
        dxn2 = K.linear_dgrad(dh, Wi_b, Wi_t)
        dWi = K.linear_wgrad(dh, xn2) if n_i else None
        del dh, h, xn2
        gx32, gx16, dw_mn = K.layernorm_bwd(dxn2, x_mid, w_mn, mean_m, rstd_m, gx32, True)
        del dxn2, x_mid
        ad = (geo.drop.attn, geo.drop.seed, i) if geo.drop is not None and geo.drop.attn else None
        gt16 = gx16 if ad is None else K.dropout_f32(gx32, ad[0], ad[1], i, K.SITE_ATTN_OUT, geo.S, geo.cu, bf16_only=True)
        do = K.linear_dgrad(gt16, Wo_b, Wo_t)
        dWo = K.linear_wgrad(gt16, o) if n_o else None
        del gt16
        dqkv = _attn_backward(geo, i, qkv, o, do, lse, ad)
        del do, o, qkv
        dWqkv = K.linear_wgrad(dqkv, xn) if n_qkv else None
        if i == 0:
            dw_an = None
            if need[2]:
                dxn = K.linear_dgrad(dqkv, Wqkv_b, Wqkv_t)
                gx32, _ = K.add_f32(gx32, dxn, want_bf16=False)
            _hand_upstream(geo, gx32, None)
        elif need[2] or n_an:
            dxn = K.linear_dgrad(dqkv, Wqkv_b, Wqkv_t)
            gx32, gx16, dw_an = K.layernorm_bwd(dxn, x, w_an, mean_a, rstd_a, gx32, True)
            _hand_upstream(geo, gx32, gx16)
        else:
            dw_an = None
        grads = [dWqkv, dWo, dw_mn, dWi, dWo2] if i == 0 else [dw_an, dWqkv, dWo, dw_mn, dWi, dWo2]
        out = [(gw if gw.dtype == dt else gw.to(dt)) if (nd and gw is not None) else None for gw, dt, nd in zip(grads, ctx.wdtypes, need[3:])]
        return (None, None, gx32 if need[2] else None, *out)


class _FinalNormFn(torch.autograd.Function):

    @staticmethod
    def forward(ctx, geo: _Geometry, x: Tensor, norm_w: Tensor):
        w = _f32(norm_w.detach())
        if geo.bf16:
            _, y, mean, rstd = K.layernorm_fwd(x, w, geo.eps, False, True, geo.save)
            if geo.save:
                ctx.geo, ctx.pack, ctx.wdtype = geo, (x, w, mean, rstd), norm_w.dtype
            return y
        y, _, mean, rstd = K.layernorm_fwd(x, w, geo.eps, True, False, geo.save)
        if geo.save:
            ctx.geo, ctx.pack, ctx.wdtype = geo, (x, w, mean, rstd), norm_w.dtype
        return y

    @staticmethod
    def backward(ctx, dy: Tensor):
        x, w, mean, rstd = ctx.pack
        if ctx.geo.bf16:
            _, g, dw = K.layernorm_bwd(dy.to(torch.bfloat16).contiguous(), x, w, mean, rstd, None, False, inplace=False, bf16_only=True)
            ctx.pack = None
            _hand_upstream(ctx.geo, g, g)
            return None, g if ctx.needs_input_grad[1] else None, dw.to(ctx.wdtype) if ctx.needs_input_grad[2] else None
        gx32, gx16, dw = K.layernorm_bwd(dy.contiguous(), x, w, mean, rstd, None, True, inplace=False)
        ctx.pack = None
        _hand_upstream(ctx.geo, gx32, gx16)
        return None, gx32 if ctx.needs_input_grad[1] else None, dw.to(ctx.wdtype) if ctx.needs_input_grad[2] else None


class _EmbedLNFn(torch.autograd.Function):

    @staticmethod
    def forward(ctx, ids: Tensor, table: Tensor, norm_w: Tensor, eps: float, padding_idx: int, slot: Optional[Tensor],
                audio_rows: Optional[Tensor], bf16: bool = False):
        w = _f32(norm_w.detach())
        tab = table.detach()
        ar = audio_rows.detach().contiguous() if audio_rows is not None else None
        if bf16:
            _, y, mean, rstd = K.embed_ln_fwd(ids, tab, w, eps, slot, ar, want_bf16=True, want_f32=False)
        else:
            y, _, mean, rstd = K.embed_ln_fwd(ids, tab, w, eps, slot, ar)
        ctx.pack = (ids, tab, w, mean, rstd, slot, ar, padding_idx)
        ctx.dtypes = (table.dtype, norm_w.dtype, audio_rows.dtype if audio_rows is not None else None)
        return y

    @staticmethod
    def backward(ctx, dy: Tensor):
        ids, tab, w, mean, rstd, slot, ar, padding_idx = ctx.pack
        d_table, d_audio, dw = K.embed_ln_bwd(dy.contiguous(), ids, tab, w, mean, rstd, padding_idx, slot, ar,
                                              want_table_grad=ctx.needs_input_grad[1])
        td, wd, ad = ctx.dtypes
        if d_table is not None and d_table.dtype != td:
            d_table = d_table.to(td)
        if d_audio is not None and d_audio.dtype != ad:
            d_audio = d_audio.to(ad)
        return None, d_table, dw.to(wd), None, None, None, d_audio, None


class _DropPlan:

    __slots__ = ("seed", "embedding", "attn", "mlp")

    def __init__(self, seed: int, embedding: int, attn: int, mlp: int):
        self.seed, self.embedding, self.attn, self.mlp = seed, embedding, attn, mlp
# ... 356 lines not shown
```

cm3p_amd/isa_check.py:

```python
from __future__ import annotations

import os
import re
import subprocess

CSRC = os.path.join(os.path.dirname(os.path.abspath(__file__)), "csrc")


class IsaCheckError(AssertionError):
    pass


def _need(cond, msg):
    if not cond:
        raise IsaCheckError(msg)


def compile_isa(src: str, flags: list[str], hipcc: str | None = None) -> str:
    hipcc = hipcc or os.environ.get("HIPCC", "/opt/rocm/bin/hipcc")
    cmd = [hipcc, *[f for f in flags if f != "-Wall"], "-S", "--cuda-device-only", "-o", "-", os.path.join(CSRC, src)]
    return subprocess.run(cmd, check=True, capture_output=True, text=True).stdout


def kernel_bodies(isa: str, name: str) -> dict[str, str]:
    isa = re.sub(r"^\s*;.*\n", "", isa, flags=re.M)
    out = {}
    for m in re.finditer(r"^(_ZN\S*" + re.escape(name) + r"\S*):", isa, re.M):
        out[m.group(1)] = isa[m.start():isa.index(".Lfunc_end", m.start())]
    return out


def no_scratch(isa: str, what: str):
    for key in ("private_segment_fixed_size", "vgpr_spill_count"):
        for m in re.finditer(r"\." + key + r":\s*(\d+)", isa):
            _need(int(m.group(1)) == 0, f"{what}: {key} = {m.group(1)} (a spilled register turns ring loads into synchronous round trips "
                                         "and breaks the counted vmcnt waits)")


def loops(body: str):
    labels = {m.group(1): m.start() for m in re.finditer(r"^(\.LBB\d+_\d+):", body, re.M)}
    for m in re.finditer(r"s_c?branch\S*\s+(\.LBB\d+_\d+)", body):
        if m.group(1) in labels and labels[m.group(1)] < m.start():
            yield m.group(1), body[labels[m.group(1)]:m.start()]


def check_gemm8p(isa: str):
    no_scratch(isa, "gemm8p.hip")
    bodies = kernel_bodies(isa, "gemm8p_kernel")
    _need(len(bodies) >= 36, f"gemm8p.hip: {len(bodies)} kernel instances found")
    for sym, body in bodies.items():
        m = re.search(r"gemm8p_kernelILb[01]ELb[01]ELi\d+ELb([01])EEEv", sym)
        _need(m, f"{sym}: template arguments not recognised")
        rebal = m.group(1) == "1"
        n = 2 if rebal else 1
        ring = [seg for _, seg in loops(body) if seg.count("v_mfma_f32_16x16x32_bf16") == 64 * n]
        _need(ring, f"{sym}: steady-state k-loop ({64 * n} MFMAs) not found")
        seg = min(ring, key=len)
        dma = len(re.findall(r"\bglobal_load_lds_dwordx4\b", seg))
        _need(dma == 8 * n, f"{sym}: {dma} LDS-DMA instructions per loop iteration, expected {8 * n}")
        _need(seg.count("s_barrier") == 8 * n, f"{sym}: {seg.count('s_barrier')} barriers per loop iteration, expected {8 * n}")
        waits = re.findall(r"s_waitcnt vmcnt\((\d+)\)", seg)
        want = ["10", "6"] * n if rebal else ["6"]
        _need(sorted(waits) == sorted(want) and all(a != b for a, b in zip(waits, waits[1:])),
              f"{sym}: vector-memory waits in the k-loop are {waits}, expected alternating {want}")
        for m in re.finditer(r"s_waitcnt vmcnt\((?:6|10)\)", seg):
            _need(re.match(r"\s*s_barrier", seg[m.end():]), f"{sym}: a counted wait is not directly in front of a barrier")
        if rebal:
            runs = [len(re.findall(r"\bglobal_load_lds_dwordx4\b", part)) for part in re.split(r"s_waitcnt vmcnt\(\d+\)", seg)]
            after = runs[1:-1] + [runs[-1] + runs[0]]
            _need(after == [6 if w == "6" else 2 for w in waits], f"{sym}: LDS-DMA instructions behind the counted waits {waits} are {after}")
        _need("scratch_" not in seg and not re.search(r"\b(buffer_|flat_|global_load_dword|global_store)", seg),
              f"{sym}: stray memory instruction in the k-loop")
        lg = re.findall(r"s_waitcnt lgkmcnt\((8|15)\)\s*\n\s*s_barrier", seg)
        _need(len(lg) == (0 if rebal else 1), f"{sym}: the B-lo retire wait (lgkmcnt(8|15) in front of phase 1's barrier) appears {len(lg)} times")
        for m in re.finditer(r"v_mfma_f32_16x16x32_bf16 (v\[\d+:\d+\]), v\[\d+:\d+\], v\[\d+:\d+\], (\S+)", seg):
            _need(m.group(1) == m.group(2), f"{sym}: an accumulating MFMA of the k-loop has D != C ({m.group(0)})")
        total = len(re.findall(r"\bglobal_load_lds_dwordx4\b", body))
        _need(total == 14 + 16 * n, f"{sym}: {total} LDS-DMA instructions in the kernel, expected {14 + 16 * n}")
        _need(body.count("s_waitcnt vmcnt(0)") >= 1, f"{sym}: the final drain of the ring is missing")
        _need(re.search(r"s_nop 15\s*\n\s*s_nop 7", body), f"{sym}: the epilogue's wait states behind the asm MFMAs are missing")


def check_attention_bwd_fused(isa: str):
    no_scratch(isa, "attention_bwd_fused.hip")
    for variant in ("ILb1ELb0E", "ILb0ELb0E", "ILb1ELb1E", "ILb0ELb1E"):
        add = variant.endswith("ELb1E")
        bodies = kernel_bodies(isa, "attn_bwd_fused_kernel" + variant)
        _need(len(bodies) == 1, f"attn_bwd_fused_kernel{variant}: {len(bodies)} instances")
        sym, body = next(iter(bodies.items()))
        ring = [seg for _, seg in loops(body) if seg.count("v_mfma_f32_32x32x16_bf16") == 480]
        _need(ring, f"{sym}: unrolled six-tile ring not found")
        ring = ring[-1]
        _need("v_accvgpr_write" not in ring and "v_accvgpr_read" not in ring and "scratch_" not in ring, f"{sym}: accumulator copies / scratch in the ring")
        _need(ring.count("global_load_lds_dwordx4") == 24 and ring.count("global_load_lds_dword ") == 6, f"{sym}: LDS-DMA count per ring changed")
        stores, atomics = len(re.findall(r"\bglobal_store_dwordx4\b", ring)), len(re.findall(r"\bglobal_atomic_pk_add_bf16\b", ring))
        _need((stores, atomics) == ((0, 48) if add else (12, 0)) and len(re.findall(r"\bglobal_(load|store|atomic)_", ring)) == 30 + stores + atomics,
              f"{sym}: vector-memory instruction count per ring changed ({stores} stores, {atomics} atomics)")
        _need(not re.search(r"\bbuffer_|\bflat_", ring), f"{sym}: buffer / flat instruction in the ring")
        _need(ring.count("s_barrier") == 6, f"{sym}: barriers per ring")
        n = "21" if add else "9"
        _need(re.findall(r"s_waitcnt vmcnt\((\d+)\)", ring) == [n] * 6 and "vmcnt(0)" not in ring, f"{sym}: the ring's waits are not six vmcnt({n})")
        for m in re.finditer(r"s_barrier", ring):
            _need(f"vmcnt({n})" in ring[max(0, m.start() - 400):m.start()], f"{sym}: a barrier without its counted wait")
        _need(re.search(r"v_mfma_f32_32x32x16_bf16 v\[\d+:\d+\], a\[\d+:\d+\], v\[\d+:\d+\], v\[\d+:\d+\]", ring), f"{sym}: dQ MFMA form")
        _need(ring.count("v_exp_f32") == 384 and len(re.findall(r"v_exp_f32_e64 v\d+, v\d+ clamp", ring)) == 384, f"{sym}: exponentials / clamp")


def hot_path(lines: list[str], lo: int, hi: int):
    labels = {m.group(1): i for i, l in enumerate(lines) if (m := re.match(r"^(\.LBB\d+_\d+):", l))}
    i = lo
    while i <= hi:
        l = lines[i]
        yield i, l
        m = re.search(r"s_cbranch_\S+\s+(\.LBB\d+_\d+)", l)
        if m and m.group(1) in labels and i < labels[m.group(1)] <= hi:
            i = labels[m.group(1)]
            continue
        if m and labels.get(m.group(1)) == lo:
            return
        i += 1


def check_attention_fwd(isa: str):
    no_scratch(isa, "attention_fwd.hip")
    for mask in (False, True):
        bodies = kernel_bodies(isa, "attn_fwd_g_kernelILi4ELb%dE" % int(mask))
        _need(len(bodies) == 1, f"attn_fwd_g_kernel<4, {mask}>: {len(bodies)} instances")
        sym, body = next(iter(bodies.items()))
        rings = [seg for _, seg in loops(body) if seg.count("v_mfma_f32_32x32x16_bf16") == 256]
        _need(len(rings) == 2, f"{sym}: {len(rings)} four-tile loops (256 MFMAs) found, expected the all-visible sweep and the masked sweep")
        nd = "5" if mask else "4"
        lines = body.split("\n")
# ... 66 lines not shown
```

cm3p_amd/kernels.py:

```python
from __future__ import annotations

import math
import os
from typing import Optional

import torch

from . import _lib
from ._lib import ADD_A_BF16, BF16, GEMM_F32_TILED, POOL_PACKED, EPI_BF16, EPI_BF16_GEGLU_BWD, EPI_BF16_GEGLU_FWD, EPI_BF16_RESID, EPI_F32, EPI_F32_RESID, F32, call, dt, ptr, query, stream

Tensor = torch.Tensor

_lib.HBM_BOUND_TAGS.update({"cm3p_layernorm_fwd", "cm3p_layernorm_bwd", "cm3p_geglu_fwd", "cm3p_geglu_bwd", "attn_bwd_prep_kernel [global]",
                            "attn_bwd_dq_reduce_kernel [global]", "attn_bwd_prep_kernel [global, varlen]", "attn_bwd_dq_reduce_kernel [global, varlen]"})


def _empty(shape, dtype, like: Tensor) -> Tensor:
    return torch.empty(shape, dtype=dtype, device=like.device)


def layernorm_fwd(x: Tensor, weight: Tensor, eps: float, want_f32: bool, want_bf16: bool, want_stats: bool = True):
    rows, H = x.shape
    y32 = _empty((rows, H), torch.float32, x) if want_f32 else None
    y16 = _empty((rows, H), torch.bfloat16, x) if want_bf16 else None
    mean = _empty((rows,), torch.float32, x) if want_stats else None
    rstd = _empty((rows,), torch.float32, x) if want_stats else None
    call("cm3p_layernorm_fwd", ptr(x), dt(x), ptr(weight, torch.float32), ptr(y32), ptr(y16), ptr(mean, torch.float32), ptr(rstd, torch.float32), rows, H, eps, stream(),
         work=float(rows) * H * (x.element_size() + (4 if want_f32 else 0) + (2 if want_bf16 else 0)))
    return y32, y16, mean, rstd


def layernorm_bwd(dy: Tensor, x: Tensor, weight: Tensor, mean: Tensor, rstd: Tensor, dres: Optional[Tensor],
                  want_bf16: bool, inplace: bool = True, bf16_only: bool = False):
    rows, H = x.shape
    if bf16_only:
        dx32 = None
        dx16 = dres if (inplace and dres is not None and dres.dtype == torch.bfloat16) else _empty((rows, H), torch.bfloat16, x)
    else:
        dx32 = dres if (inplace and dres is not None and dres.dtype == torch.float32) else _empty((rows, H), torch.float32, x)
        dx16 = _empty((rows, H), torch.bfloat16, x) if want_bf16 else None
    nblk = query("cm3p_layernorm_bwd_blocks", rows)
    part = _empty((nblk, H), torch.float32, x)
    dw = _empty((H,), torch.float32, x)
    call("cm3p_layernorm_bwd", ptr(dy), dt(dy), ptr(x), dt(x), ptr(weight, torch.float32), ptr(mean, torch.float32), ptr(rstd, torch.float32), ptr(dres),
         dt(dres) if dres is not None else F32, ptr(dx32), ptr(dx16), ptr(part), ptr(dw), rows, H, stream(),
         work=float(rows) * H * (dy.element_size() + x.element_size() + (dres.element_size() if dres is not None else 0)
                                 + (4 if dx32 is not None else 0) + (2 if dx16 is not None else 0)))
    return dx32, dx16, dw


def embed_ln_fwd(ids: Tensor, table: Tensor, weight: Tensor, eps: float, slot: Optional[Tensor] = None,
                 override: Optional[Tensor] = None, want_bf16: bool = False, want_f32: bool = True):
    T = ids.numel()
    H = table.shape[1]
    if not (want_f32 or want_bf16):
        raise ValueError("embed_ln_fwd: no output requested")
    y32 = _empty((T, H), torch.float32, table) if want_f32 else None
    y16 = _empty((T, H), torch.bfloat16, table) if want_bf16 else None
    mean = _empty((T,), torch.float32, table)
    rstd = _empty((T,), torch.float32, table)
    call("cm3p_embed_ln_fwd", ptr(ids, torch.int64), ptr(table), dt(table), ptr(slot, torch.int32), ptr(override), dt(override) if override is not None else F32,
         ptr(weight, torch.float32), ptr(y32), ptr(y16), ptr(mean, torch.float32), ptr(rstd, torch.float32), T, H, eps, table.shape[0], stream())
    return y32, y16, mean, rstd


def embed_ln_bwd(dy: Tensor, ids: Tensor, table: Tensor, weight: Tensor, mean: Tensor, rstd: Tensor, padding_idx: int,
                 slot: Optional[Tensor] = None, override: Optional[Tensor] = None, want_table_grad: bool = True):
    T = ids.numel()
    V, H = table.shape
    if want_table_grad and T > 0 and os.environ.get("CM3P_EMBED_BWD", "sorted") != "atomic":
        return _embed_ln_bwd_sorted(dy, ids, table, weight, mean, rstd, padding_idx, slot, override)
    d_table = torch.zeros((V, H), dtype=torch.float32, device=table.device) if want_table_grad else None
    d_ovr = torch.zeros(override.shape, dtype=torch.float32, device=table.device) if override is not None else None
    nblk = query("cm3p_layernorm_bwd_blocks", T)
    part = _empty((nblk, H), torch.float32, table)
    dw = _empty((H,), torch.float32, table)
    call("cm3p_embed_ln_bwd", ptr(dy), dt(dy), ptr(ids, torch.int64), ptr(table), dt(table), ptr(slot, torch.int32), ptr(override),
         dt(override) if override is not None else F32, ptr(weight, torch.float32), ptr(mean, torch.float32), ptr(rstd, torch.float32), ptr(d_table), ptr(d_ovr), ptr(part), ptr(dw),
         T, H, padding_idx, V, stream())
    return d_table, d_ovr, dw


def _embed_ln_bwd_sorted(dy, ids, table, weight, mean, rstd, padding_idx, slot, override):
    T = ids.numel()
    V, H = table.shape
    dev = table.device
    chunk = query("cm3p_embed_ln_bwd_sorted_chunk")
    flat = ids.reshape(-1).to(torch.int64).contiguous()
    order, run_of = token_order(flat, V, chunk)
    R = min(T, V + 3 + T // chunk)
    run_rows = _empty((R, H), torch.float32, table)
    run_ids = torch.empty((R,), dtype=torch.int64, device=dev)
# ... 183 lines not shown
def _drop_abi(drop: Optional[tuple]) -> tuple:
    if drop is None:
        return "", (), ">"
    thr, seed, layer = drop
    return "_dropout", (layer, thr, seed), ", DropCfg>"


def _attn_fwd_name(window: int, prescaled: bool, masked: bool, S: int, nh: int, targs_end: str = ">") -> str:
    if targs_end == ">" and query("cm3p_attn_fwd_impl", S, nh, window, int(prescaled)):
        return "attn_fwd_g_kernel<4, " + ("true>" if masked else "false>")
    return "attn_fwd_kernel<1, %s, " + ("true" if window >= 0 else "false") + targs_end


def attn_fwd(qkv: Tensor, key_mask: Optional[Tensor], B: int, S: int, nh: int, window: int, scale: float, prescaled: bool = False,
             drop: Optional[tuple] = None):
    out = torch.empty((B * S, nh * 64), dtype=torch.bfloat16, device=qkv.device)
    lse = torch.empty((B, nh, S), dtype=torch.float32, device=qkv.device)
    keys = S if window < 0 else min(S, 2 * window + 1)
    sfx, drop_args, targs_end = _drop_abi(drop)
    call("cm3p_attn_fwd" + sfx, ptr(qkv), ptr(out), ptr(lse, torch.float32), ptr(key_mask, torch.uint8), B, S, nh, window, scale, int(prescaled),
         *drop_args, stream(), tag=_attn_tag(_attn_fwd_name(window, prescaled, key_mask is not None, S, nh, targs_end), window, prescaled),
         work=4.0 * B * nh * S * keys * 64)
    return out, lse


HD_MFMA_SIZES = (96, 128)


def attn_generic_supported(head_dim: int) -> bool:
    return bool(query("cm3p_attn_generic_supported", int(head_dim)))


def _attn_hd_prof(names: tuple, products: int, B: int, S: int, nh: int, hd: int, window: int) -> dict:
    if hd not in HD_MFMA_SIZES:
        return {}
    keys = S if window < 0 else min(S, 2 * window + 1)
    return dict(tag=_attn_tag(" + ".join(f"{n}<{hd}>" for n in names), window, False), work=2.0 * products * B * nh * S * keys * hd)


def rope_apply_generic_(qkv: Tensor, cos: Tensor, sin: Tensor, B: int, S: int, nh: int, hd: int, per_batch: bool, inverse: bool = False):
    call("cm3p_rope_apply_generic", ptr(qkv, torch.bfloat16), ptr(cos, torch.float32), ptr(sin, torch.float32), B, S, nh, hd, S if per_batch else 0, int(inverse), stream())
    return qkv


def attn_fwd_generic(qkv: Tensor, key_mask: Optional[Tensor], B: int, S: int, nh: int, hd: int, window: int, scale: float,
                     drop: Optional[tuple] = None):
    out = torch.empty((B * S, nh * hd), dtype=torch.bfloat16, device=qkv.device)
    lse = torch.empty((B, nh, S), dtype=torch.float32, device=qkv.device)
    sfx, drop_args, _ = _drop_abi(drop)
    prof = {} if drop is not None else _attn_hd_prof(("attn_hd_fwd_kernel",), 2, B, S, nh, hd, window)
    call("cm3p_attn_fwd_generic" + sfx, ptr(qkv, torch.bfloat16), ptr(out), ptr(lse, torch.float32), ptr(key_mask, torch.uint8), B, S, nh, hd, window, scale,
         *drop_args, stream(), **prof)
    return out, lse


def attn_bwd_generic(qkv: Tensor, out: Tensor, dout: Tensor, lse: Tensor, key_mask: Optional[Tensor], B: int, S: int, nh: int, hd: int,
                     window: int, scale: float, drop: Optional[tuple] = None) -> Tensor:
    dqkv = torch.empty_like(qkv)
    delta = torch.empty_like(lse)
    sfx, drop_args, _ = _drop_abi(drop)
    prof = {} if drop is not None else _attn_hd_prof(("attn_hd_dq_kernel", "attn_hd_dkv_kernel"), 4, B, S, nh, hd, window)
    call("cm3p_attn_bwd_generic" + sfx, ptr(qkv, torch.bfloat16), ptr(out, torch.bfloat16), ptr(dout, torch.bfloat16), ptr(lse, torch.float32), ptr(delta),
         ptr(dqkv), ptr(key_mask, torch.uint8), B, S, nh, hd, window, scale, *drop_args, stream(), **prof)
    return dqkv


def attn_probs(qkv: Tensor, lse: Tensor, key_mask: Optional[Tensor], B: int, S: int, nh: int, window: int, scale: float, prescaled: bool = False) -> Tensor:
    probs = torch.empty((B, nh, S, S), dtype=torch.float32, device=qkv.device)
    call("cm3p_attn_probs", ptr(qkv), ptr(lse, torch.float32), ptr(key_mask, torch.uint8), ptr(probs), B, S, nh, window, scale, int(prescaled), stream())
    return probs


ATTN_BWD_DQ, ATTN_BWD_DKV = 1, 2


def _attn_tag(fmt: str, window: int, prescaled: bool, varlen: bool = False) -> str:
    name = fmt % ("true" if prescaled else "false") if "%s" in fmt else fmt
    return f"{name} [{'global' if window < 0 else 'local'}{', varlen' if varlen else ''}]"


ATTN_BWD_FUSED_PREP, ATTN_BWD_FUSED_MAIN, ATTN_BWD_FUSED_REDUCE = 1, 2, 4
ATTN_BWD_FUSED_MAIN_EVEN, ATTN_BWD_FUSED_MAIN_ODD = 8, 16
ATTN_BWD_FUSED_MAIN_ADD1 = 32
_fused_ws: dict = {}


_other_caches: list = []


def release_workspaces() -> None:
    _fused_ws.clear()
    for c in _other_caches:
        c.clear()


def _attn_bwd_fused(qkv, out, dout, lse, key_mask, cu, B, S, total, nh, scale, rope, per_batch, prescaled) -> Tensor:
    dqkv = torch.empty_like(qkv)
    cos, sin = rope if rope is not None else (None, None)
    need = query("cm3p_attn_bwd_fused_workspace_bytes", B, S, nh)
    key = (qkv.device.index, torch.cuda.current_stream(qkv.device).cuda_stream)
    ws = _fused_ws.get(key)
    if ws is None or ws.numel() < need:
        ws = _fused_ws[key] = torch.empty(need, dtype=torch.uint8, device=qkv.device)
    varlen = cu is not None
    rows = total if varlen else B * S
    fl = 2.0 * B * nh * S * S * 64
    nkb = -(-S // 256)
    G = query("cm3p_attn_bwd_fused_slab_group", S)
    n_store = -(-nkb // G)
    slabs = float(need) * 2.0 / G
    adds = [(ATTN_BWD_FUSED_MAIN_ADD1 << (p - 1), "attn_bwd_fused_kernel<%s, true>", 4.0 * fl * len(range(p, nkb, G)) / nkb)
            for p in range(1, min(G, nkb))]
    for stage, name, work in (
        (ATTN_BWD_FUSED_PREP, "attn_bwd_prep_kernel", 2.0 * rows * nh * 64 * 2 + 12.0 * rows * nh),
        (ATTN_BWD_FUSED_MAIN_EVEN, "attn_bwd_fused_kernel<%s, false>", 4.0 * fl * n_store / nkb),
        *adds,
        (ATTN_BWD_FUSED_REDUCE, "attn_bwd_dq_reduce_kernel", slabs + rows * nh * 64 * 2.0),
    ):
        call("cm3p_attn_bwd_fused", ptr(qkv), ptr(out), ptr(dout), ptr(lse, torch.float32), ptr(dqkv), ptr(key_mask, torch.uint8),
             ptr(cu, torch.int32), B, S, total if varlen else 0, nh, scale, ptr(cos, torch.float32), ptr(sin, torch.float32),
             S if (per_batch and not varlen) else 0, stage, int(prescaled), ptr(ws), ws.numel(), stream(),
             tag=_attn_tag(name, -1, prescaled, varlen), work=None if varlen else work)
    return dqkv


def attn_bwd(qkv: Tensor, out: Tensor, dout: Tensor, lse: Tensor, key_mask: Optional[Tensor], B: int, S: int, nh: int,
             window: int, scale: float, rope: Optional[tuple] = None, per_batch: bool = False, prescaled: bool = False,
             drop: Optional[tuple] = None) -> Tensor:
    if drop is None and window < 0:
        return _attn_bwd_fused(qkv, out, dout, lse, key_mask, None, B, S, 0, nh, scale, rope, per_batch, prescaled)
    dqkv = torch.empty_like(qkv)
    delta = torch.empty_like(lse)
    keys = S if window < 0 else min(S, 2 * window + 1)
    cos, sin = rope if rope is not None else (None, None)
    sfx, drop_args, targs_end = _drop_abi(drop)
    for stage, name, products in ((ATTN_BWD_DQ, "attn_bwd_dq_kernel<%s", 1), (ATTN_BWD_DKV, "attn_bwd_dkv_kernel<%s", 3)):
        call("cm3p_attn_bwd" + sfx, ptr(qkv), ptr(out), ptr(dout), ptr(lse, torch.float32), ptr(delta), ptr(dqkv), ptr(key_mask, torch.uint8), B, S, nh,
             window, scale, ptr(cos, torch.float32), ptr(sin, torch.float32), S if per_batch else 0, stage, int(prescaled), *drop_args, stream(),
             tag=_attn_tag(name + targs_end, window, prescaled), work=None if drop is not None else 2.0 * products * B * nh * S * keys * 64)
    return dqkv


def attn_fwd_varlen(qkv: Tensor, cu: Tensor, B: int, max_s: int, nh: int, window: int, scale: float, prescaled: bool = False,
                    drop: Optional[tuple] = None):
    total = qkv.shape[0]
    out = torch.empty((total, nh * 64), dtype=torch.bfloat16, device=qkv.device)
    lse = torch.empty((nh, total), dtype=torch.float32, device=qkv.device)
    sfx, drop_args, targs_end = _drop_abi(drop)
    call("cm3p_attn_fwd" + sfx + "_varlen", ptr(qkv), ptr(out), ptr(lse, torch.float32), ptr(cu, torch.int32), B, max_s, total, nh, window, scale,
         int(prescaled), *drop_args, stream(), tag=_attn_tag(_attn_fwd_name(window, prescaled, False, max_s, nh, targs_end), window, prescaled, True))
    return out, lse


def attn_bwd_varlen(qkv: Tensor, out: Tensor, dout: Tensor, lse: Tensor, cu: Tensor, B: int, max_s: int, nh: int, window: int,
                    scale: float, rope: Optional[tuple] = None, prescaled: bool = False, drop: Optional[tuple] = None) -> Tensor:
    if drop is None and window < 0:
        return _attn_bwd_fused(qkv, out, dout, lse, None, cu, B, max_s, qkv.shape[0], nh, scale, rope, False, prescaled)
    dqkv = torch.empty_like(qkv)
    delta = torch.empty_like(lse)
    cos, sin = rope if rope is not None else (None, None)
    sfx, drop_args, targs_end = _drop_abi(drop)
    for stage, name in ((ATTN_BWD_DQ, "attn_bwd_dq_kernel<%s"), (ATTN_BWD_DKV, "attn_bwd_dkv_kernel<%s")):
        call("cm3p_attn_bwd" + sfx + "_varlen", ptr(qkv), ptr(out), ptr(dout), ptr(lse, torch.float32), ptr(delta), ptr(dqkv), ptr(cu, torch.int32), B,
             max_s, qkv.shape[0], nh, window, scale, ptr(cos, torch.float32), ptr(sin, torch.float32), stage, int(prescaled), *drop_args, stream(),
             tag=_attn_tag(name + targs_end, window, prescaled, True))
    return dqkv


def _rows_as_f32(src: Tensor) -> Tensor:
    return src.view(torch.float32) if src.dtype == torch.bfloat16 else src


def gather_rows(src: Tensor, idx: Tensor) -> Tensor:
    s32 = _rows_as_f32(src)
    out = torch.empty((idx.numel(), s32.shape[1]), dtype=torch.float32, device=src.device)
    if idx.numel() == 0:
        return out.view(src.dtype)
    call("cm3p_gather_rows_f32", ptr(s32), ptr(idx, torch.int64), ptr(out), idx.numel(), s32.shape[1], stream())
    return out.view(src.dtype)


def scatter_rows(src: Tensor, idx: Tensor, rows: int) -> Tensor:
    s32 = _rows_as_f32(src)
    out = torch.zeros((rows, s32.shape[1]), dtype=torch.float32, device=src.device)
    if idx.numel() == 0:
        return out.view(src.dtype)
    call("cm3p_scatter_rows_f32", ptr(s32), ptr(idx, torch.int64), ptr(out), idx.numel(), s32.shape[1], stream())
    return out.view(src.dtype)


def geglu_fwd(h: Tensor) -> Tensor:
    T, I2 = h.shape
    g = torch.empty((T, I2 // 2), dtype=torch.bfloat16, device=h.device)
    call("cm3p_geglu_fwd", ptr(h), ptr(g), T, I2 // 2, stream(), work=6.0 * T * (I2 // 2))
    return g


def gemm_geglu_supported(T: int, I: int, Kd: int) -> bool:
    code = query("cm3p_gemm_route", T, 2 * I, Kd, Kd, Kd, 1, 1, EPI_GEGLU, 1, 0, 0)
    return code >= 0 and (code & 3) == _GEMM_RING


def geglu_interleave_index(I: int, device) -> Tensor:
    n = torch.arange(2 * I, device=device)
    r = n % 64
    j = (n // 64) * 32 + r % 32
    return torch.where(r < 32, j, I + j)


def gemm_geglu(x: Tensor, w_interleaved: Tensor) -> Tensor:
    T, Kd = x.shape
    I = w_interleaved.shape[0] // 2
    a = _empty((T, I), torch.bfloat16, x)
    call("cm3p_gemm_geglu", ptr(x), ptr(w_interleaved), ptr(a), T, I, Kd, stream(),
         tag=_gemm_tag(T, 2 * I, Kd, True, True, EPI_GEGLU, 1, kernel=_GEMM_RING), work=2.0 * T * 2 * I * Kd)
    return a


def mlp_geglu_fused_supported(T: int, I: int, H: int) -> bool:
    fwd = query("cm3p_gemm_route", T, 2 * I, H, H, H, 1, 1, EPI_BF16_GEGLU_FWD, 1, 0, 0)
    bwd = query("cm3p_gemm_route", T, I, H, H, H, 1, 1, EPI_BF16_GEGLU_BWD, 1, 0, 0)
    return fwd >= 0 and (fwd & 3) == _GEMM_RING and bwd >= 0 and (bwd & 3) == _GEMM_RING


def linear_geglu_fwd(x: Tensor, w_interleaved: Tensor):
    T, Kd = x.shape
    N = w_interleaved.shape[0]
    h = _empty((T, N), torch.bfloat16, x)
    a = _empty((T, N // 2), torch.bfloat16, x)
    call("cm3p_gemm_bf16", ptr(x), ptr(w_interleaved), ptr(h), None, T, N, Kd, Kd, Kd, N, 1, 1, EPI_BF16_GEGLU_FWD, 1, ptr(a), stream(),
         tag=_gemm_tag(T, N, Kd, True, True, EPI_BF16_GEGLU_FWD, 1), work=2.0 * T * N * Kd)
    return h, a


def linear_dgrad_geglu_bwd(dy: Tensor, w_t: Tensor, h_interleaved: Tensor) -> Tensor:
    T, Kd = dy.shape
    I = w_t.shape[0]
    dh = torch.empty_like(h_interleaved)
    call("cm3p_gemm_bf16", ptr(dy), ptr(w_t), ptr(dh), ptr(h_interleaved), T, I, Kd, Kd, Kd, 2 * I, 1, 1, EPI_BF16_GEGLU_BWD, 1, None, stream(),
         tag=_gemm_tag(T, I, Kd, True, True, EPI_BF16_GEGLU_BWD, 1), work=2.0 * T * I * Kd)
    return dh


def geglu_bwd(dg: Tensor, h: Tensor) -> Tensor:
    dh = torch.empty_like(h)
    call("cm3p_geglu_bwd", ptr(dg), ptr(h), ptr(dh), h.shape[0], h.shape[1] // 2, stream(), work=10.0 * h.shape[0] * (h.shape[1] // 2))
    return dh


SITE_EMBED, SITE_ATTN_PROBS, SITE_ATTN_OUT, SITE_MLP = 0, 1, 2, 3


def dropout_threshold(p: float) -> int:
    return int(math.floor(float(p) * 65536.0 + 0.5))


def dropout_scale(thr: int) -> float:
    return 0.0 if thr >= 65536 else float(torch.tensor(65536.0) / torch.tensor(float(65536 - thr)))


def _drop_rows(S: int, cu: Optional[Tensor]):
    return (S, None, 0) if cu is None else (S, ptr(cu, torch.int32), cu.numel() - 1)


def dropout_f32(x: Tensor, thr: int, seed: int, layer: int, site: int, S: int, cu: Optional[Tensor] = None, resid: Optional[Tensor] = None,
                bf16_only: bool = False) -> Tensor:
    rows, H = x.shape
    y = torch.empty(x.shape, dtype=torch.bfloat16 if bf16_only else torch.float32, device=x.device)
    call("cm3p_dropout_f32", ptr(x, torch.float32), ptr(resid, torch.float32), None if bf16_only else ptr(y), ptr(y) if bf16_only else None, rows, H,
         *_drop_rows(S, cu), layer, site, thr, seed, stream())
    return y


def geglu_fwd_dropout(h: Tensor, thr: int, seed: int, layer: int, S: int, cu: Optional[Tensor] = None) -> Tensor:
    T, I2 = h.shape
    g = torch.empty((T, I2 // 2), dtype=torch.bfloat16, device=h.device)
    call("cm3p_geglu_fwd_dropout", ptr(h, torch.bfloat16), ptr(g), T, I2 // 2, *_drop_rows(S, cu), layer, thr, seed, stream())
    return g


def geglu_bwd_dropout(dg: Tensor, h: Tensor, thr: int, seed: int, layer: int, S: int, cu: Optional[Tensor] = None) -> Tensor:
    dh = torch.empty_like(h)
    call("cm3p_geglu_bwd_dropout", ptr(dg, torch.bfloat16), ptr(h, torch.bfloat16), ptr(dh), h.shape[0], h.shape[1] // 2, *_drop_rows(S, cu),
         layer, thr, seed, stream())
    return dh


def dropout_keep(n2: int, n1: int, n0: int, layer: int, site: int, thr: int, seed: int, device) -> Tensor:
    keep = torch.empty((n2, n1, n0), dtype=torch.uint8, device=device)
    call("cm3p_dropout_keep", ptr(keep), n2, n1, n0, layer, site, thr, seed, stream())
    return keep


def philox4x32_10_host(ctr, key):
    import numpy as np

    c = np.ascontiguousarray(ctr, dtype=np.uint32).reshape(-1, 4)
    k = np.ascontiguousarray(key, dtype=np.uint32).reshape(-1, 2)
    if c.shape[0] != k.shape[0]:
        raise ValueError("one key per counter")
    out = np.empty_like(c)
    _lib._check(query("cm3p_philox4x32_10_host", c.ctypes.data, k.ctypes.data, out.ctypes.data, c.shape[0]), "cm3p_philox4x32_10_host")
    return out


def gelu_fwd(x: Tensor) -> Tensor:
    y = torch.empty_like(x)
    call("cm3p_gelu_fwd", ptr(x), ptr(y), x.numel(), stream())
    return y


def gelu_bwd(dy: Tensor, x: Tensor) -> Tensor:
    dx = torch.empty_like(x)
    call("cm3p_gelu_bwd", ptr(dy), ptr(x), ptr(dx), x.numel(), stream())
    return dx


def im2col_k3(x: Tensor, token_major: bool, B: int, C: int, T_in: int, stride: int):
    T_out = (T_in - 1) // stride + 1
    p = torch.empty((B * T_out, C * 3), dtype=torch.bfloat16, device=x.device)
    call("cm3p_im2col_k3", ptr(x, torch.bfloat16 if token_major else torch.float32), int(token_major), ptr(p), B, C, T_in, T_out, stride, stream())
    return p, T_out


# ... 196 lines not shown
```

include/cm3p_hip.h:

```cpp
#ifndef CM3P_HIP_H
#define CM3P_HIP_H

#include <stdint.h>

#ifdef __cplusplus
extern "C" {
#endif

#define CM3P_OK 0
#define CM3P_ERR_INVALID (-1)
#define CM3P_ERR_LAUNCH (-2)
#define CM3P_ERR_INTERNAL (-3)

#define CM3P_F32 0
#define CM3P_BF16 1

#define CM3P_ABI_VERSION 20
int cm3p_abi_version(void);

int cm3p_layernorm_fwd(const void* x, int x_dtype, const float* weight, float* y_f32, void* y_bf16, float* mean,
                       float* rstd, int64_t rows, int H, float eps, void* stream);

int cm3p_layernorm_bwd_blocks(int64_t rows);

int cm3p_layernorm_bwd(const void* dy, int dy_dtype, const void* x, int x_dtype, const float* weight, const float* mean,
                       const float* rstd, const void* dres, int dres_dtype, float* dx_f32, void* dx_bf16, float* dw_partial,
                       float* dw, int64_t rows, int H, void* stream);

int cm3p_embed_ln_fwd(const int64_t* ids, const void* table, int table_dtype, const int32_t* slot,
                      const void* override_rows, int override_dtype, const float* weight, float* y_f32, void* y_bf16,
                      float* mean, float* rstd, int64_t T, int H, float eps, int64_t vocab, void* stream);

int cm3p_embed_ln_bwd(const void* dy, int dy_dtype, const int64_t* ids, const void* table, int table_dtype, const int32_t* slot,
                      const void* override_rows, int override_dtype, const float* weight, const float* mean,
                      const float* rstd, float* d_table, float* d_override, float* dw_partial, float* dw, int64_t T, int H,
                      int64_t padding_idx, int64_t vocab, void* stream);

int cm3p_embed_ln_bwd_sorted_chunk(void);
int cm3p_embed_ln_bwd_sorted(const void* dy, int dy_dtype, const int64_t* ids, const int64_t* order, const int32_t* run_of, const void* table,
                             int table_dtype, const int32_t* slot, const void* override_rows, int override_dtype, const float* weight,
                             const float* mean, const float* rstd, float* d_table, float* d_override, float* run_rows, int64_t* run_ids,
                             float* dw_partial, float* dw, int64_t T, int H, int64_t padding_idx, int64_t vocab, void* stream);

int64_t cm3p_token_order_workspace_ints(int64_t T, int64_t vocab);
int cm3p_token_order(const int64_t* ids, int64_t T, int64_t vocab, int64_t* order, int32_t* run_of, int32_t* workspace, void* stream);

int cm3p_audio_slots(const int64_t* ids, int64_t T, int64_t audio_token_id, int32_t* slot, int32_t* count, void* stream);

#define CM3P_EPI_BF16 0
#define CM3P_EPI_F32 1
#define CM3P_EPI_F32_RESID 2
#define CM3P_EPI_F32_BIAS 5
#define CM3P_EPI_BF16_RESID 7
#define CM3P_EPI_BF16_GEGLU_FWD 9
#define CM3P_EPI_BF16_GEGLU_BWD 10
int cm3p_gemm_bf16(const void* A, const void* B, void* C, const float* R, int64_t M, int64_t N, int64_t K, int64_t lda,
                   int64_t ldb, int64_t ldc, int a_kc, int b_kc, int epilogue, int split_k, float* workspace, void* stream);

int cm3p_gemm8p_set_grid(int workgroups);
int cm3p_gemm8p_get_grid(void);

int cm3p_build_ablation_flags(void);

int cm3p_debug_set_dma_audit(void* buf);

int cm3p_qkv_gemm_rope(const void* x, const void* Wqkv, void* qkv, int64_t M, int64_t N, int64_t K, const float* cos_tab,
                       const float* sin_tab, int S, int per_batch, int rope_cols, float q_scale, void* stream);

int cm3p_gemm_wgrad_splits(int64_t M, int64_t N, int64_t K);

int cm3p_gemm_route(int64_t M, int64_t N, int64_t K, int64_t lda, int64_t ldb, int a_kc, int b_kc, int epilogue, int split_k,
                    int rope_cols, int batch);

int cm3p_cast_f32_bf16(const float* x, void* y, int64_t n, void* stream);
int cm3p_cast_f32_bf16_t(const float* x, void* y, void* y_t, int64_t rows, int64_t cols, void* stream);
int cm3p_cast_f32_bf16_t_multi(const int64_t* table, int n, int64_t total_blocks, void* stream);
#define CM3P_ADD_A_BF16 16
int cm3p_add_f32(const void* a, const void* b, int b_dtype, float* y_f32, void* y_bf16, int64_t n, void* stream);

int cm3p_rope_table(const int64_t* position_ids, int64_t n_pos, const float* inv_freq, int half_dim, float* cos_out,
                    float* sin_out, void* stream);
int cm3p_rope_apply(void* qkv, const float* cos_tab, const float* sin_tab, int B, int S, int nh, int64_t pos_batch_stride,
                    int inverse, void* stream);

int cm3p_attn_fwd(const void* qkv, void* out, float* lse, const uint8_t* key_mask, int B, int S, int nh, int window,
                  float scale, int q_prescaled, void* stream);
int cm3p_attn_fwd_impl(int S, int nh, int window, int q_prescaled);

int cm3p_attn_probs(const void* qkv, const float* lse, const uint8_t* key_mask, float* probs, int B, int S, int nh, int window, float scale,
                    int q_prescaled, void* stream);
#define CM3P_ATTN_BWD_DQ 1
#define CM3P_ATTN_BWD_DKV 2
int cm3p_attn_bwd(const void* qkv, const void* out, const void* dout, const float* lse, float* delta, void* dqkv,
                  const uint8_t* key_mask, int B, int S, int nh, int window, float scale, const float* cos_tab,
                  const float* sin_tab, int64_t pos_batch_stride, int stages, int q_prescaled, void* stream);

int cm3p_attn_generic_supported(int head_dim);
int cm3p_attn_fwd_generic(const void* qkv, void* out, float* lse, const uint8_t* key_mask, int B, int S, int nh, int head_dim, int window,
                          float scale, void* stream);
int cm3p_attn_bwd_generic(const void* qkv, const void* out, const void* dout, const float* lse, float* delta, void* dqkv,
                          const uint8_t* key_mask, int B, int S, int nh, int head_dim, int window, float scale, void* stream);
int cm3p_attn_fwd_generic_dropout(const void* qkv, void* out, float* lse, const uint8_t* key_mask, int B, int S, int nh, int head_dim,
                                  int window, float scale, int layer, int thr, uint64_t seed, void* stream);
int cm3p_attn_bwd_generic_dropout(const void* qkv, const void* out, const void* dout, const float* lse, float* delta, void* dqkv,
                                  const uint8_t* key_mask, int B, int S, int nh, int head_dim, int window, float scale, int layer, int thr,
                                  uint64_t seed, void* stream);
int cm3p_rope_apply_generic(void* qkv, const float* cos_tab, const float* sin_tab, int B, int S, int nh, int head_dim, int64_t pos_batch_stride,
                            int inverse, void* stream);

#define CM3P_ATTN_BWD_FUSED_PREP 1
#define CM3P_ATTN_BWD_FUSED_MAIN 2
#define CM3P_ATTN_BWD_FUSED_REDUCE 4
#define CM3P_ATTN_BWD_FUSED_MAIN_EVEN 8
#define CM3P_ATTN_BWD_FUSED_MAIN_ODD 16
#define CM3P_ATTN_BWD_FUSED_MAIN_ADD1 32
int64_t cm3p_attn_bwd_fused_workspace_bytes(int B, int S, int nh);
int cm3p_attn_bwd_fused_slab_group(int S);
int cm3p_attn_bwd_fused(const void* qkv, const void* out, const void* dout, const float* lse, void* dqkv, const uint8_t* key_mask,
                        const int* cu_seqlens, int B, int S, int64_t total, int nh, float scale, const float* cos_tab,
                        const float* sin_tab, int64_t pos_batch_stride, int stages, int q_prescaled, void* workspace,
                        int64_t workspace_bytes, void* stream);

int cm3p_attn_fwd_dropout(const void* qkv, void* out, float* lse, const uint8_t* key_mask, int B, int S, int nh, int window, float scale,
                          int q_prescaled, int layer, int thr, uint64_t seed, void* stream);
int cm3p_attn_bwd_dropout(const void* qkv, const void* out, const void* dout, const float* lse, float* delta, void* dqkv,
                          const uint8_t* key_mask, int B, int S, int nh, int window, float scale, const float* cos_tab,
                          const float* sin_tab, int64_t pos_batch_stride, int stages, int q_prescaled, int layer, int thr, uint64_t seed,
                          void* stream);
int cm3p_attn_fwd_dropout_varlen(const void* qkv, void* out, float* lse, const int* cu_seqlens, int B, int max_seqlen, int64_t total, int nh,
                                 int window, float scale, int q_prescaled, int layer, int thr, uint64_t seed, void* stream);
int cm3p_attn_bwd_dropout_varlen(const void* qkv, const void* out, const void* dout, const float* lse, float* delta, void* dqkv,
                                 const int* cu_seqlens, int B, int max_seqlen, int64_t total, int nh, int window, float scale,
                                 const float* cos_tab, const float* sin_tab, int stages, int q_prescaled, int layer, int thr, uint64_t seed,
                                 void* stream);

int cm3p_geglu_fwd(const void* h, void* g, int64_t T, int I, void* stream);

int cm3p_gemm_geglu(const void* x, const void* w_interleaved, void* a, int64_t T, int64_t I, int64_t K, void* stream);
int cm3p_geglu_bwd(const void* dg, const void* h, void* dh, int64_t T, int I, void* stream);
int cm3p_dropout_f32(const float* x, const float* resid, float* y_f32, void* y_bf16, int64_t rows, int H, int S, const int* cu_seqlens,
                     int n_seqs, int layer, int site, int thr, uint64_t seed, void* stream);
int cm3p_geglu_fwd_dropout(const void* h, void* g, int64_t T, int I, int S, const int* cu_seqlens, int n_seqs, int layer, int thr,
                           uint64_t seed, void* stream);
int cm3p_geglu_bwd_dropout(const void* dg, const void* h, void* dh, int64_t T, int I, int S, const int* cu_seqlens, int n_seqs, int layer,
                           int thr, uint64_t seed, void* stream);
int cm3p_dropout_keep(uint8_t* keep, int n2, int n1, int n0, int layer, int site, int thr, uint64_t seed, void* stream);
int cm3p_philox4x32_10_host(const uint32_t* ctr, const uint32_t* key, uint32_t* out, int64_t n);

int cm3p_gelu_fwd(const void* x, void* y, int64_t n, void* stream);
int cm3p_gelu_bwd(const void* dy, const void* x, void* dx, int64_t n, void* stream);

int cm3p_im2col_k3(const void* x, int x_token_major, void* patches, int B, int C, int T_in, int T_out, int stride, void* stream);
int cm3p_col2im_k3(const void* dpatches, void* dx, int B, int C, int T_in, int T_out, int stride, void* stream);
int cm3p_bias_gelu_fwd(const float* z, const float* bias, void* a_bf16, float* a_f32, int64_t R, int C, void* stream);
int cm3p_bias_gelu_bwd_blocks(int64_t R);
int cm3p_bias_gelu_bwd(const void* da, int da_dtype, const float* z, const float* bias, void* dz_bf16, float* db_partial,
                       float* dbias, int64_t R, int C, void* stream);

#define CM3P_POOL_PACKED 2
int cm3p_pool_chunks(int S);
int cm3p_pool_fwd(const void* h, int h_dtype, const int64_t* mask, float* pooled, float* partial, float* count, int Bn, int S, int H,
                  int cls, void* stream);
int cm3p_pool_bwd(const float* dpooled, const int64_t* mask, const float* count, void* dh, int dh_dtype, int Bn, int S, int H,
                  int cls, void* stream);

#define CM3P_GEMM_F32_TILED 2
int cm3p_gemm_f32(const float* A, const float* B, float* C, int M, int N, int K, int64_t a_rs, int64_t a_cs, int64_t b_rs,
                  int64_t b_cs, int64_t ldc, float alpha, int accumulate, void* stream);
int cm3p_l2norm_fwd(const float* x, float* y, float* norm, int rows, int D, void* stream);
int cm3p_l2norm_bwd(const float* dy, const float* y, const float* norm, float* dx, int rows, int D, void* stream);
int cm3p_cross_entropy(const float* logits, int rows, int cols, int64_t row_stride, int64_t col_stride,
                       const int64_t* row_offset, const int64_t* target, float grad_scale, float* loss_rows, float* dlogits,
                       void* stream);
int cm3p_scale_exp(const float* x, const float* log_scale, float* y, int64_t n, void* stream);
int cm3p_scale_by(const float* x, const float* scale, float* y, int64_t n, void* stream);
int cm3p_dot_f32(const float* a, const float* b, float* out, int64_t n, void* stream);
int cm3p_sum_f32(const float* x, float* out, int64_t n, float scale, int accumulate, void* stream);
int cm3p_cross_entropy_masked(const float* logits, int64_t rows, int cols, int64_t row_stride, const int64_t* target,
                              int64_t ignore_index, float grad_scale, const float* inv_count, float* loss_rows, float* dlogits,
                              void* stream);
int cm3p_inv_valid_count(const int64_t* target, int64_t n, int64_t ignore_index, float* inv_count, void* stream);
int cm3p_ce_masked_stats(const float* logits, int64_t rows, int cols, int64_t row_stride, const int64_t* target, int64_t ignore_index,
                         float* loss_rows, float* lse_rows, void* stream);
int cm3p_ce_masked_dlogits_blocks(int64_t rows);
int cm3p_ce_masked_dlogits_bf16(const float* logits, int64_t rows, int cols, int64_t row_stride, const int64_t* target, int64_t ignore_index,
                                const float* lse_rows, const float* scale_a, const float* scale_b, void* dlogits_bf16, float* partial,
                                float* colsum, void* stream);
int cm3p_add_bias_f32(float* x, const float* bias, int64_t rows, int cols, void* stream);
int cm3p_colsum_blocks(int64_t rows);
int cm3p_colsum_f32(const float* x, float* partial, float* out, int64_t rows, int cols, void* stream);

int cm3p_pointwise_loss(const float* x, const float* y, float* out, float* dx, int64_t n, int kind, void* stream);

int cm3p_first_zero_index(const int64_t* classes, int B, int V, int64_t* idx, void* stream);

int cm3p_attn_fwd_varlen(const void* qkv, void* out, float* lse, const int* cu_seqlens, int B, int max_seqlen, int64_t total,
                         int nh, int window, float scale, int q_prescaled, void* stream);
int cm3p_attn_bwd_varlen(const void* qkv, const void* out, const void* dout, const float* lse, float* delta, void* dqkv,
// ... 23 lines not shown
```

Before: 197.2 pairs/s.

## Fuse attention-backward delta (rowsum O·dO) into the Wo dgrad GEMM epilogue

Adds a new GEMM epilogue that, while storing dO from the Wo dgrad GEMM, also loads O and computes the per-row dot product O·dO, writing the negated delta directly into the fused attention-backward stats workspace. The attention backward then runs a light prep kernel that only writes scaled LSE values instead of re-reading O and dO. This removes a full read pass over O and dO per global layer, at the cost of extra loads and LDS traffic in the GEMM epilogue and more coupling between the GEMM and attention workspace layouts. It is enabled by default for global, non-dropout, head-dim-64 layers when the ring GEMM route is chosen.

```diff
diff --git a/cm3p_amd/_lib.py b/cm3p_amd/_lib.py
--- a/cm3p_amd/_lib.py
+++ b/cm3p_amd/_lib.py
@@ -12,6 +12,7 @@
 GEMM_F32_TILED = 2
 EPI_BF16, EPI_F32, EPI_F32_RESID, EPI_F32_BIAS, EPI_BF16_RESID = 0, 1, 2, 5, 7
 EPI_BF16_GEGLU_FWD, EPI_BF16_GEGLU_BWD = 9, 10
+EPI_BF16_DELTA = 11
 ABI_VERSION = 20
 
 _HERE = os.path.dirname(os.path.abspath(__file__))
diff --git a/cm3p_amd/csrc/attention_bwd_fused.hip b/cm3p_amd/csrc/attention_bwd_fused.hip
--- a/cm3p_amd/csrc/attention_bwd_fused.hip
+++ b/cm3p_amd/csrc/attention_bwd_fused.hip
@@ -67,20 +67,31 @@
     if (row < S) {
         const uint16_t* po = o_rows + (sv.row0 + row) * ldo + head * 64 + part * 16;
         const uint16_t* pg = d_o + (sv.row0 + row) * ldo + head * 64 + part * 16;
-#pragma unroll
-        for (int h = 0; h < 2; ++h) {
-            const bf16x8 a = gload_frag8(po + 8 * h), g = gload_frag8(pg + 8 * h);
-#pragma unroll
-            for (int j = 0; j < 8; ++j) acc += (float)a[j] * (float)g[j];
-        }
-    }
-    acc += __shfl_xor(acc, 1, 64);
-    acc += __shfl_xor(acc, 2, 64);
+        const bf16x8 a[2] = {gload_frag8(po), gload_frag8(po + 8)}, g[2] = {gload_frag8(pg), gload_frag8(pg + 8)};
+        acc = delta_prep_quarter(a, g);
+    }
+    acc = delta_prep_join(acc);
     if (part == 0) {
         float* st = stat_ws + (((int64_t)b * nh + head) * gridDim.x + t) * 128;
         const bool ok = row < S;
         st[tid >> 2] = ok ? lse[sv.stat0 + row] * lse_mul : kNegInf;
         st[64 + (tid >> 2)] = ok ? -acc : 0.f;
+    }
+}
+
+__global__ __launch_bounds__(256) void attn_bwd_prep_lse_kernel(const float* __restrict__ lse, float* __restrict__ stat_ws, int S, int tiles,
+                                                                int64_t nrows, float lse_mul) {
+    const int64_t idx = (int64_t)blockIdx.x * 256 + threadIdx.x;
+    if (idx >= nrows) return;
+    const int r = (int)(idx & 63);
+    const int64_t tile = idx >> 6, bh = tile / tiles;
+    const int row = (int)(tile - bh * tiles) * 64 + r;
+    float* st = stat_ws + tile * 128;
+    if (row < S) {
+        st[r] = lse[bh * S + row] * lse_mul;
+    } else {
+        st[r] = kNegInf;
+        st[64 + r] = 0.f;
     }
 }
 
@@ -666,6 +677,8 @@
 
 }
 
+int cm3p_attn_bwd_fused_stat_tiles(int S) { return (S + 63) / 64 + kFPadTiles; }
+
 extern "C" {
 
 int cm3p_attn_bwd_fused_slab_group(int S) {
@@ -685,7 +698,8 @@
                         const float* sin_tab, int64_t pos_batch_stride, int stages, int q_prescaled, void* workspace,
                         int64_t workspace_bytes, void* stream) {
     CM3P_REQUIRE((cos_tab == nullptr) == (sin_tab == nullptr));
-    CM3P_REQUIRE(stages >= 1 && stages <= 255);
+    CM3P_REQUIRE(stages >= 1 && (stages & ~(255 | CM3P_ATTN_BWD_FUSED_PREP_LSE)) == 0);
+    CM3P_REQUIRE(!(stages & CM3P_ATTN_BWD_FUSED_PREP_LSE) || (!cu_seqlens && !(stages & CM3P_ATTN_BWD_FUSED_PREP)));
     CM3P_REQUIRE(qkv && out && dout && lse && dqkv && workspace && B > 0 && S > 0 && nh > 0 && scale > 0.f);
     CM3P_REQUIRE(cm3p_aligned16(qkv) && cm3p_aligned16(out) && cm3p_aligned16(dout) && cm3p_aligned16(dqkv) && cm3p_aligned16(workspace));
     if (cu_seqlens) CM3P_REQUIRE(total > 0 && key_mask == nullptr && pos_batch_stride == 0);
@@ -706,7 +720,13 @@
                                                                           lse_mul, vl);
         if (hipGetLastError() != hipSuccess) return CM3P_ERR_LAUNCH;
     }
-    const bool run_even = stages & (CM3P_ATTN_BWD_FUSED_MAIN | CM3P_ATTN_BWD_FUSED_MAIN_EVEN);
+    if (stages & CM3P_ATTN_BWD_FUSED_PREP_LSE) {
+        const float lse_mul = pre ? -kLog2e : -1.0f / scale;
+        const int64_t nrows = (int64_t)B * nh * (NT + kFPadTiles) * 64;
+        attn_bwd_prep_lse_kernel<<<(unsigned)((nrows + 255) / 256), 256, 0, s>>>(lse, stat_ws, S, NT + kFPadTiles, nrows, lse_mul);
+        if (hipGetLastError() != hipSuccess) return CM3P_ERR_LAUNCH;
+    }
+    const bool run_even =stages & (CM3P_ATTN_BWD_FUSED_MAIN | CM3P_ATTN_BWD_FUSED_MAIN_EVEN);
     const bool run_odd = stages & (CM3P_ATTN_BWD_FUSED_MAIN | CM3P_ATTN_BWD_FUSED_MAIN_ODD);
     if (run_even || run_odd || (stages & (7 * CM3P_ATTN_BWD_FUSED_MAIN_ADD1))) {
         static Cm3pDevOnce once;
diff --git a/cm3p_amd/csrc/attn_common.h b/cm3p_amd/csrc/attn_common.h
--- a/cm3p_amd/csrc/attn_common.h
+++ b/cm3p_amd/csrc/attn_common.h
@@ -63,6 +63,20 @@
     __device__ __forceinline__ int64_t pos0(int b, int64_t pos_batch_stride) const { return packed ? row0 : (int64_t)b * pos_batch_stride; }
 };
 
+__device__ __forceinline__ float delta_prep_quarter(const bf16x8 (&o)[2], const bf16x8 (&g)[2]) {
+    float acc = 0.f;
+#pragma unroll
+    for (int h = 0; h < 2; ++h)
+#pragma unroll
+        for (int j = 0; j < 8; ++j) acc += (float)o[h][j] * (float)g[h][j];
+    return acc;
+}
+__device__ __forceinline__ float delta_prep_join(float acc) {
+    acc += __shfl_xor(acc, 1, 64);
+    acc += __shfl_xor(acc, 2, 64);
+    return acc;
+}
+
 __device__ __forceinline__ f32x16 mfma32(bf16x8 a, bf16x8 b, f32x16 c) {
     return __builtin_amdgcn_mfma_f32_32x32x16_bf16(a, b, c, 0, 0, 0);
 }
diff --git a/cm3p_amd/csrc/common.h b/cm3p_amd/csrc/common.h
--- a/cm3p_amd/csrc/common.h
+++ b/cm3p_amd/csrc/common.h
@@ -26,7 +26,9 @@
     const uint16_t* Rb = nullptr;
     float alpha = 1.f, beta = 0.f;
     void* C2 = nullptr;
-};
+    int dl_S = 0, dl_tiles = 0;
+};
+int cm3p_attn_bwd_fused_stat_tiles(int S);
 
 #ifndef CM3P_NT
 #define CM3P_NT 7
@@ -283,14 +285,15 @@
         case CM3P_EPI_BF16_RESID: return f(std::integral_constant<int, CM3P_EPI_BF16_RESID>{});
         case CM3P_EPI_BF16_GEGLU_FWD: return f(std::integral_constant<int, CM3P_EPI_BF16_GEGLU_FWD>{});
         case CM3P_EPI_BF16_GEGLU_BWD: return f(std::integral_constant<int, CM3P_EPI_BF16_GEGLU_BWD>{});
+        case CM3P_EPI_BF16_DELTA: return f(std::integral_constant<int, CM3P_EPI_BF16_DELTA>{});
         default: return CM3P_ERR_INTERNAL;
     }
 }
-constexpr bool cm3p_epi_is_geglu(int epi) {
-    return epi == CM3P_EPI_BF16_GEGLU || epi == CM3P_EPI_BF16_GEGLU_FWD || epi == CM3P_EPI_BF16_GEGLU_BWD;
+constexpr bool cm3p_epi_is_ring_only(int epi) {
+    return epi == CM3P_EPI_BF16_GEGLU || epi == CM3P_EPI_BF16_GEGLU_FWD || epi == CM3P_EPI_BF16_GEGLU_BWD || epi == CM3P_EPI_BF16_DELTA;
 }
 constexpr bool cm3p_gemm_pair_exists(bool a_kc, bool b_kc, int epi) {
-    return (epi != CM3P_EPI_BF16_ROPE && epi != CM3P_EPI_F32_BIAS && !cm3p_epi_is_geglu(epi)) || (a_kc && b_kc);
+    return (epi != CM3P_EPI_BF16_ROPE && epi != CM3P_EPI_F32_BIAS && !cm3p_epi_is_ring_only(epi)) || (a_kc && b_kc);
 }
 
 template <bool INVERSE>
diff --git a/cm3p_amd/csrc/gemm.hip b/cm3p_amd/csrc/gemm.hip
--- a/cm3p_amd/csrc/gemm.hip
+++ b/cm3p_amd/csrc/gemm.hip
@@ -196,7 +196,7 @@
 }
 
 template <bool A_KC, bool B_KC, int EPI>
-constexpr bool has_instance = cm3p_gemm_pair_exists(A_KC, B_KC, EPI) && !cm3p_epi_is_geglu(EPI);
+constexpr bool has_instance = cm3p_gemm_pair_exists(A_KC, B_KC, EPI) && !cm3p_epi_is_ring_only(EPI);
 
 int launch128(const GemmRoute& r, const GemmCall& g, hipStream_t s) {
     const int tiles_m = (int)((g.M + BM - 1) / BM), tiles_n = (int)((g.N + BN - 1) / BN);
@@ -231,7 +231,7 @@
                                     int split_k, int rope_cols, int batch) {
     GemmRoute r{CM3P_GEMM_128, false, 1, K};
     const bool batched = epi == CM3P_EPI_BF16_AXPBY;
-    if (M <= 0 || N <= 0 || K <= 0 || split_k < 1 || epi < 0 || epi > CM3P_EPI_BF16_GEGLU_BWD || epi == 8  || batched != (batch > 0) ||
+    if (M <= 0 || N <= 0 || K <= 0 || split_k < 1 || epi < 0 || epi > CM3P_EPI_BF16_DELTA || epi == 8  || batched != (batch > 0) ||
         !cm3p_gemm_pair_exists(a_kc, b_kc, epi)) {
         r.kernel = CM3P_ERR_INVALID;
         return r;
@@ -253,6 +253,8 @@
     } else if (epi == CM3P_EPI_BF16_GEGLU_FWD || epi == CM3P_EPI_BF16_GEGLU_BWD) {
         const int64_t cols = epi == CM3P_EPI_BF16_GEGLU_FWD ? 64 : 32;
         r.kernel = (big && N % cols == 0 && ring_ok && split_k == 1 && !no_ring && !small_only) ? CM3P_GEMM_RING : CM3P_ERR_INVALID;
+    } else if (epi == CM3P_EPI_BF16_DELTA) {
+        r.kernel = (big && N % 64 == 0 && M < (int64_t(1) << 31) && ring_ok && split_k == 1 && !no_ring && !small_only) ? CM3P_GEMM_RING : CM3P_ERR_INVALID;
     } else if (batched) {
         const bool filled = M * N * batch * 10 >= items * 65536 * 7;
         big = big && filled && (a_kc || !b_kc) && ring_ok && !no_ring;
@@ -353,16 +355,20 @@
                    int64_t ldb, int64_t ldc, int a_kc, int b_kc, int epilogue, int split_k, float* workspace, void* stream) {
     CM3P_REQUIRE(A && B && C && M > 0 && N > 0 && K > 0);
     const bool geglu_fwd = epilogue == CM3P_EPI_BF16_GEGLU_FWD, geglu_bwd = epilogue == CM3P_EPI_BF16_GEGLU_BWD;
+    const bool delta = epilogue == CM3P_EPI_BF16_DELTA;
+    const int dl_S = delta ? split_k : 0;
+    if (delta) split_k = 1;
     CM3P_REQUIRE((epilogue >= CM3P_EPI_BF16 && epilogue <= CM3P_EPI_F32_RESID) || epilogue == CM3P_EPI_F32_BIAS || epilogue == CM3P_EPI_BF16_RESID ||
-                 geglu_fwd || geglu_bwd);
+                 geglu_fwd || geglu_bwd || delta);
     CM3P_REQUIRE(cm3p_aligned16(A) && cm3p_aligned16(B) && cm3p_aligned16(C));
     CM3P_REQUIRE(lda % 8 == 0 && ldb % 8 == 0 && ldc % 4 == 0 && N % 4 == 0);
     CM3P_REQUIRE(a_kc ? (K % 8 == 0 && lda >= K) : (M % 8 == 0 && lda >= M));
     CM3P_REQUIRE(b_kc ? (K % 8 == 0 && ldb >= K) : (N % 8 == 0 && ldb >= N));
     CM3P_REQUIRE(ldc >= N);
-    CM3P_REQUIRE((epilogue != CM3P_EPI_F32_RESID && epilogue != CM3P_EPI_F32_BIAS && epilogue != CM3P_EPI_BF16_RESID && !geglu_bwd) || (R && cm3p_aligned16(R)));
+    CM3P_REQUIRE((epilogue != CM3P_EPI_F32_RESID && epilogue != CM3P_EPI_F32_BIAS && epilogue != CM3P_EPI_BF16_RESID && !geglu_bwd && !delta) || (R && cm3p_aligned16(R)));
     CM3P_REQUIRE(!geglu_fwd || (workspace && cm3p_aligned16(workspace) && ldc == N && N % 64 == 0 && split_k == 1));
     CM3P_REQUIRE(!geglu_bwd || (ldc == 2 * N && N % 32 == 0 && split_k == 1));
+    CM3P_REQUIRE(!delta || (workspace && cm3p_aligned16(workspace) && ldc == N && N % 64 == 0 && dl_S > 0 && M % dl_S == 0));
     CM3P_REQUIRE(epilogue != CM3P_EPI_BF16_RESID || (N % 8 == 0 && ldc % 8 == 0));
     CM3P_REQUIRE(split_k >= 1 && (split_k == 1 || (epilogue == CM3P_EPI_F32 && workspace && cm3p_aligned16(workspace) && ldc == N)));
     const GemmRoute r = cm3p_gemm_route_of(M, N, K, lda, ldb, a_kc != 0, b_kc != 0, epilogue, split_k, 0, 0);
@@ -370,6 +376,11 @@
     hipStream_t s = static_cast<hipStream_t>(stream);
     GemmCall g{A, B, C, R, M, N, K, lda, ldb, ldc, a_kc != 0, b_kc != 0, epilogue};
     if (geglu_fwd) g.bt.C2 = workspace;
+    if (delta) {
+        g.bt.C2 = workspace;
+        g.bt.dl_S = dl_S;
+        g.bt.dl_tiles = cm3p_attn_bwd_fused_stat_tiles(dl_S);
+    }
     if (r.splits > 1) {
         g.C = workspace;
         g.c_split_stride = M * N;
diff --git a/cm3p_amd/csrc/gemm256.hip b/cm3p_amd/csrc/gemm256.hip
--- a/cm3p_amd/csrc/gemm256.hip
+++ b/cm3p_amd/csrc/gemm256.hip
@@ -356,7 +356,7 @@
 }
 
 template <bool A_KC, bool B_KC, int EPI>
-constexpr bool has_instance = cm3p_gemm_pair_exists(A_KC, B_KC, EPI) && !cm3p_epi_is_geglu(EPI) && EPI != CM3P_EPI_BF16_AXPBY;
+constexpr bool has_instance = cm3p_gemm_pair_exists(A_KC, B_KC, EPI) && !cm3p_epi_is_ring_only(EPI) && EPI != CM3P_EPI_BF16_AXPBY;
 
 }
 
diff --git a/cm3p_amd/csrc/gemm8p.hip b/cm3p_amd/csrc/gemm8p.hip
--- a/cm3p_amd/csrc/gemm8p.hip
+++ b/cm3p_amd/csrc/gemm8p.hip
@@ -2,6 +2,7 @@
 
 #include <type_traits>
 
+#include "attn_common.h"
 #include "common.h"
 
 #ifndef CM3P_G8P_ABL
@@ -502,6 +503,60 @@
                 }
                 if constexpr (CM3P_G8P_ABL & 1) asm volatile("" ::"v"(oa.x), "v"(ob.x));
             }
+        } else if constexpr (EPI == CM3P_EPI_BF16_DELTA) {
+            char* Cb = reinterpret_cast<char*>(static_cast<uint16_t*>(Cv) + mw * ldc + nw);
+            const char* Ob = reinterpret_cast<const char*>(reinterpret_cast<const uint16_t*>(R) + mw * ldc + nw);
+            const uint32_t ldcb = (uint32_t)ldc * 2;
+            const uint32_t S = (uint32_t)bt.dl_S, nh = (uint32_t)(N >> 6), head = (uint32_t)(nw >> 6);
+            const uint32_t b0 = (uint32_t)mw / S, s0 = (uint32_t)mw - b0 * S;
+            const int srow = lane >> 2, part = lane & 3;
+            const bool wave_cols = FULL || nw < N;
+            u32x4 on[8][2];
+#pragma unroll
+            for (int i4 = 0; i4 < 8; ++i4) {
+                const bool ok = wave_cols && (FULL || mw + i4 * 16 + srow < M);
+                const char* p = Ob + (uint32_t)(i4 * 16 + srow) * ldcb + part * 32;
+                const u32x4 zero = {0u, 0u, 0u, 0u};
+                if constexpr (CM3P_G8P_ABL & 1) {
+                    asm volatile("" : "=v"(on[i4][0]), "=v"(on[i4][1]) : "v"(p));
+                } else {
+                    on[i4][0] = ok ? __builtin_bit_cast(u32x4, gload16<(CM3P_NT & 64) != 0>(p)) : zero;
+                    on[i4][1] = ok ? __builtin_bit_cast(u32x4, gload16<(CM3P_NT & 64) != 0>(p + 16)) : zero;
+                }
+            }
+#pragma unroll
+            for (int i4 = 0; i4 < 8; ++i4) {
+                char* eb = ebuf + (i4 & 1) * 2048;
+#pragma unroll
+                for (int j4 = 0; j4 < 4; ++j4) {
+                    const f32x4 a = acc[i4][j4];
+                    const int row = lane & 15, s8 = (j4 * 4 + (lane >> 4)) ^ ((row & 7) << 1);
+                    *reinterpret_cast<uint2*>(eb + row * 128 + s8 * 8) = uint2{pack_bf16x2(a.x, a.y), pack_bf16x2(a.z, a.w)};
+                }
+                G8P_LANE_XCHG_FENCE();
+                const int r0 = lane >> 3, r1 = 8 + (lane >> 3), ch = lane & 7;
+                const u32x4 x0 = *reinterpret_cast<const u32x4*>(eb + r0 * 128 + ((ch ^ (r0 & 7)) << 4));
+                const u32x4 x1 = *reinterpret_cast<const u32x4*>(eb + r1 * 128 + ((ch ^ (r1 & 7)) << 4));
+                const bf16x8 gs[2] = {__builtin_bit_cast(bf16x8, *reinterpret_cast<const u32x4*>(eb + srow * 128 + (((2 * part) ^ (srow & 7)) << 4))),
+                                      __builtin_bit_cast(bf16x8, *reinterpret_cast<const u32x4*>(eb + srow * 128 + (((2 * part + 1) ^ (srow & 7)) << 4)))};
+                G8P_LANE_XCHG_FENCE();
+                const bool col_ok = FULL || nw + ch * 8 < N;
+                if (FULL || (col_ok && mw + i4 * 16 + r0 < M)) G8P_GLOBAL(gstore16<(CM3P_NT & 1) != 0>(Cb + (uint32_t)(i4 * 16 + r0) * ldcb + ch * 16, x0));
+                if (FULL || (col_ok && mw + i4 * 16 + r1 < M)) G8P_GLOBAL(gstore16<(CM3P_NT & 1) != 0>(Cb + (uint32_t)(i4 * 16 + r1) * ldcb + ch * 16, x1));
+                if constexpr (CM3P_G8P_ABL & 1) asm volatile("" ::"v"(x0), "v"(x1));
+                const bf16x8 os[2] = {__builtin_bit_cast(bf16x8, on[i4][0]), __builtin_bit_cast(bf16x8, on[i4][1])};
+                const float v = -delta_prep_join(delta_prep_quarter(os, gs));
+                uint32_t x = s0 + (uint32_t)(i4 * 16 + srow), bb = b0;
+                if (S >= 128) {
+                    if (x >= S) x -= S, ++bb;
+                } else {
+                    bb += x / S;
+                    x %= S;
+                }
+                const int64_t at = (((int64_t)bb * nh + head) * bt.dl_tiles + (x >> 6)) * 128 + 64 + (x & 63);
+                if (part == 0 && wave_cols && (FULL || mw + i4 * 16 + srow < M)) G8P_GLOBAL(static_cast<float*>(bt.C2)[at] = v);
+                if constexpr (CM3P_G8P_ABL & 1) asm volatile("" ::"v"(v));
+            }
         } else if constexpr (EPI == CM3P_EPI_BF16_AXPBY) {
             char* Cb = reinterpret_cast<char*>(static_cast<uint16_t*>(Cv) + (int64_t)z * bt.c_stride + mw * ldc + nw);
             const char* Rb = reinterpret_cast<const char*>(bt.Rb + (int64_t)z * bt.r_stride + mw * ldc + nw);
diff --git a/cm3p_amd/encoder.py b/cm3p_amd/encoder.py
--- a/cm3p_amd/encoder.py
+++ b/cm3p_amd/encoder.py
@@ -180,14 +180,21 @@
     return x_out, (x, xn, mean_a, rstd_a, qkv, o, lse, x_mid, xn2, mean_m, rstd_m, h, g)
 
 
-def _attn_backward(geo: _Geometry, i: int, qkv: Tensor, o: Tensor, do: Tensor, lse: Tensor, ad: Optional[tuple]) -> Tensor:
+def _wo_dgrad(geo: _Geometry, i: int, g: Tensor, Wo_b: Tensor, Wo_t: Optional[Tensor], o: Tensor, ad: Optional[tuple]):
+    if os.environ.get("CM3P_DELTA_FUSED", "1") != "0" and geo.windows[i] < 0 and geo.hd == 64 and geo.cu is None \
+            and ad is None and Wo_t is not None and K.dgrad_delta_supported(g.shape[0], geo.nh * 64):
+        return K.linear_dgrad_delta(g, Wo_t, o, geo.B, geo.S, geo.nh)
+    return K.linear_dgrad(g, Wo_b, Wo_t), None
+
+
+def _attn_backward(geo: _Geometry, i: int, qkv: Tensor, o: Tensor, do: Tensor, lse: Tensor, ad: Optional[tuple], delta: Optional[Tensor] = None) -> Tensor:
     B, S, nh, window, scale = geo.B, geo.S, geo.nh, geo.windows[i], geo.hd ** -0.5
     if geo.hd != 64:
         dqkv = K.attn_bwd_generic(qkv, o, do, lse, geo.key_mask, B, S, nh, geo.hd, window, scale, drop=ad)
         return K.rope_apply_generic_(dqkv, geo.rope[i][0], geo.rope[i][1], B, S, nh, geo.hd, geo.per_batch_pos, inverse=True)
     if geo.cu is not None:
         return K.attn_bwd_varlen(qkv, o, do, lse, geo.cu, B, geo.max_s, nh, window, scale, geo.rope[i], prescaled=True, drop=ad)
-    return K.attn_bwd(qkv, o, do, lse, geo.key_mask, B, S, nh, window, scale, geo.rope[i], geo.per_batch_pos, prescaled=True, drop=ad)
+    return K.attn_bwd(qkv, o, do, lse, geo.key_mask, B, S, nh, window, scale, geo.rope[i], geo.per_batch_pos, prescaled=True, drop=ad, delta=delta)
 
 
 class _EncoderLayerFn(torch.autograd.Function):
@@ -240,9 +247,9 @@
         del dh, h, xn2
         _, g, dw_mn = K.layernorm_bwd(dxn2, x_mid, w_mn, mean_m, rstd_m, g, False, bf16_only=True)
         del dxn2, x_mid
-        do = K.linear_dgrad(g, Wo_b, Wo_t)
+        do, delta = _wo_dgrad(geo, i, g, Wo_b, Wo_t, o, None)
         dWo = K.linear_wgrad(g, o) if n_o else None
-        dqkv = _attn_backward(geo, i, qkv, o, do, lse, None)
+        dqkv = _attn_backward(geo, i, qkv, o, do, lse, None, delta)
         del do, o, qkv
         dWqkv = K.linear_wgrad(dqkv, xn) if n_qkv else None
         dw_an = None
@@ -296,10 +303,10 @@
         del dxn2, x_mid
         ad = (geo.drop.attn, geo.drop.seed, i) if geo.drop is not None and geo.drop.attn else None
         gt16 = gx16 if ad is None else K.dropout_f32(gx32, ad[0], ad[1], i, K.SITE_ATTN_OUT, geo.S, geo.cu, bf16_only=True)
-        do = K.linear_dgrad(gt16, Wo_b, Wo_t)
+        do, delta = _wo_dgrad(geo, i, gt16, Wo_b, Wo_t, o, ad)
         dWo = K.linear_wgrad(gt16, o) if n_o else None
         del gt16
-        dqkv = _attn_backward(geo, i, qkv, o, do, lse, ad)
+        dqkv = _attn_backward(geo, i, qkv, o, do, lse, ad, delta)
         del do, o, qkv
         dWqkv = K.linear_wgrad(dqkv, xn) if n_qkv else None
         if i == 0:
diff --git a/cm3p_amd/isa_check.py b/cm3p_amd/isa_check.py
--- a/cm3p_amd/isa_check.py
+++ b/cm3p_amd/isa_check.py
@@ -47,7 +47,8 @@
 def check_gemm8p(isa: str):
     no_scratch(isa, "gemm8p.hip")
     bodies = kernel_bodies(isa, "gemm8p_kernel")
-    _need(len(bodies) >= 36, f"gemm8p.hip: {len(bodies)} kernel instances found")
+    _need(len(bodies) >= 38, f"gemm8p.hip: {len(bodies)} kernel instances found")
+    _need(sum("gemm8p_kernelILb1ELb1ELi11E" in sym for sym in bodies) == 2, "gemm8p.hip: the two delta store-phase instances (epilogue 11) not found")
     for sym, body in bodies.items():
         m = re.search(r"gemm8p_kernelILb[01]ELb[01]ELi\d+ELb([01])EEEv", sym)
         _need(m, f"{sym}: template arguments not recognised")
diff --git a/cm3p_amd/kernels.py b/cm3p_amd/kernels.py
--- a/cm3p_amd/kernels.py
+++ b/cm3p_amd/kernels.py
@@ -7,7 +7,7 @@
 import torch
 
 from . import _lib
-from ._lib import ADD_A_BF16, BF16, GEMM_F32_TILED, POOL_PACKED, EPI_BF16, EPI_BF16_GEGLU_BWD, EPI_BF16_GEGLU_FWD, EPI_BF16_RESID, EPI_F32, EPI_F32_RESID, F32, call, dt, ptr, query, stream
+from ._lib import ADD_A_BF16, BF16, GEMM_F32_TILED, POOL_PACKED, EPI_BF16, EPI_BF16_DELTA, EPI_BF16_GEGLU_BWD, EPI_BF16_GEGLU_FWD, EPI_BF16_RESID, EPI_F32, EPI_F32_RESID, F32, call, dt, ptr, query, stream
 
 Tensor = torch.Tensor
 
@@ -357,6 +357,7 @@
 ATTN_BWD_FUSED_PREP, ATTN_BWD_FUSED_MAIN, ATTN_BWD_FUSED_REDUCE = 1, 2, 4
 ATTN_BWD_FUSED_MAIN_EVEN, ATTN_BWD_FUSED_MAIN_ODD = 8, 16
 ATTN_BWD_FUSED_MAIN_ADD1 = 32
+ATTN_BWD_FUSED_PREP_LSE = 512
 _fused_ws: dict = {}
 
 
@@ -369,15 +370,22 @@
         c.clear()
 
 
-def _attn_bwd_fused(qkv, out, dout, lse, key_mask, cu, B, S, total, nh, scale, rope, per_batch, prescaled) -> Tensor:
+def _fused_workspace(device, B: int, S: int, nh: int) -> Tensor:
+    need = query("cm3p_attn_bwd_fused_workspace_bytes", B, S, nh)
+    key = (device.index, torch.cuda.current_stream(device).cuda_stream)
+    ws = _fused_ws.get(key)
+    if ws is None or ws.numel() < need:
+        ws = _fused_ws[key] = torch.empty(need, dtype=torch.uint8, device=device)
+    return ws
+
+
+def _attn_bwd_fused(qkv, out, dout, lse, key_mask, cu, B, S, total, nh, scale, rope, per_batch, prescaled, delta_ws: Optional[Tensor] = None) -> Tensor:
     dqkv = torch.empty_like(qkv)
     cos, sin = rope if rope is not None else (None, None)
     need = query("cm3p_attn_bwd_fused_workspace_bytes", B, S, nh)
-    key = (qkv.device.index, torch.cuda.current_stream(qkv.device).cuda_stream)
-    ws = _fused_ws.get(key)
-    if ws is None or ws.numel() < need:
-        ws = _fused_ws[key] = torch.empty(need, dtype=torch.uint8, device=qkv.device)
+    ws = _fused_workspace(qkv.device, B, S, nh) if delta_ws is None else delta_ws
     varlen = cu is not None
+    assert delta_ws is None or (not varlen and delta_ws.numel() >= need)
     rows = total if varlen else B * S
     fl = 2.0 * B * nh * S * S * 64
     nkb = -(-S // 256)
@@ -386,8 +394,10 @@
     slabs = float(need) * 2.0 / G
     adds = [(ATTN_BWD_FUSED_MAIN_ADD1 << (p - 1), "attn_bwd_fused_kernel<%s, true>", 4.0 * fl * len(range(p, nkb, G)) / nkb)
             for p in range(1, min(G, nkb))]
+    prep = (ATTN_BWD_FUSED_PREP, "attn_bwd_prep_kernel", 2.0 * rows * nh * 64 * 2 + 12.0 * rows * nh) if delta_ws is None else \
+        (ATTN_BWD_FUSED_PREP_LSE, "attn_bwd_prep_lse_kernel", 8.0 * rows * nh)
     for stage, name, work in (
-        (ATTN_BWD_FUSED_PREP, "attn_bwd_prep_kernel", 2.0 * rows * nh * 64 * 2 + 12.0 * rows * nh),
+        prep,
         (ATTN_BWD_FUSED_MAIN_EVEN, "attn_bwd_fused_kernel<%s, false>", 4.0 * fl * n_store / nkb),
         *adds,
         (ATTN_BWD_FUSED_REDUCE, "attn_bwd_dq_reduce_kernel", slabs + rows * nh * 64 * 2.0),
@@ -401,9 +411,11 @@
 
 def attn_bwd(qkv: Tensor, out: Tensor, dout: Tensor, lse: Tensor, key_mask: Optional[Tensor], B: int, S: int, nh: int,
              window: int, scale: float, rope: Optional[tuple] = None, per_batch: bool = False, prescaled: bool = False,
-             drop: Optional[tuple] = None) -> Tensor:
+             drop: Optional[tuple] = None, delta: Optional[Tensor] = None) -> Tensor:
+    if delta is not None and (drop is not None or window >= 0):
+        raise ValueError("attn_bwd: only the global backward without dropout takes a supplied delta")
     if drop is None and window < 0:
-        return _attn_bwd_fused(qkv, out, dout, lse, key_mask, None, B, S, 0, nh, scale, rope, per_batch, prescaled)
+        return _attn_bwd_fused(qkv, out, dout, lse, key_mask, None, B, S, 0, nh, scale, rope, per_batch, prescaled, delta_ws=delta)
     dqkv = torch.empty_like(qkv)
     delta = torch.empty_like(lse)
     keys = S if window < 0 else min(S, 2 * window + 1)
@@ -515,6 +527,22 @@
     call("cm3p_gemm_bf16", ptr(dy), ptr(w_t), ptr(dh), ptr(h_interleaved), T, I, Kd, Kd, Kd, 2 * I, 1, 1, EPI_BF16_GEGLU_BWD, 1, None, stream(),
          tag=_gemm_tag(T, I, Kd, True, True, EPI_BF16_GEGLU_BWD, 1), work=2.0 * T * I * Kd)
     return dh
+
+
+def dgrad_delta_supported(T: int, H: int) -> bool:
+    code = query("cm3p_gemm_route", T, H, H, H, H, 1, 1, EPI_BF16_DELTA, 1, 0, 0)
+    return code >= 0 and (code & 3) == _GEMM_RING
+
+
+def linear_dgrad_delta(dy: Tensor, w_t: Tensor, o: Tensor, B: int, S: int, nh: int):
+    T, Kd = dy.shape
+    N = w_t.shape[0]
+    assert T == B * S and N == nh * 64 and o.shape == (T, N)
+    do = _empty((T, N), torch.bfloat16, dy)
+    ws = _fused_workspace(dy.device, B, S, nh)
+    call("cm3p_gemm_bf16", ptr(dy), ptr(w_t), ptr(do), ptr(o), T, N, Kd, Kd, Kd, N, 1, 1, EPI_BF16_DELTA, S, ptr(ws), stream(),
+         tag=_gemm_tag(T, N, Kd, True, True, EPI_BF16_DELTA, 1), work=2.0 * T * N * Kd)
+    return do, ws
 
 
 def geglu_bwd(dg: Tensor, h: Tensor) -> Tensor:
diff --git a/include/cm3p_hip.h b/include/cm3p_hip.h
--- a/include/cm3p_hip.h
+++ b/include/cm3p_hip.h
@@ -54,6 +54,7 @@
 #define CM3P_EPI_BF16_RESID 7
 #define CM3P_EPI_BF16_GEGLU_FWD 9
 #define CM3P_EPI_BF16_GEGLU_BWD 10
+#define CM3P_EPI_BF16_DELTA 11
 int cm3p_gemm_bf16(const void* A, const void* B, void* C, const float* R, int64_t M, int64_t N, int64_t K, int64_t lda,
                    int64_t ldb, int64_t ldc, int a_kc, int b_kc, int epilogue, int split_k, float* workspace, void* stream);
 
@@ -114,6 +115,7 @@
 #define CM3P_ATTN_BWD_FUSED_MAIN_EVEN 8
 #define CM3P_ATTN_BWD_FUSED_MAIN_ODD 16
 #define CM3P_ATTN_BWD_FUSED_MAIN_ADD1 32
+#define CM3P_ATTN_BWD_FUSED_PREP_LSE 512
 int64_t cm3p_attn_bwd_fused_workspace_bytes(int B, int S, int nh);
 int cm3p_attn_bwd_fused_slab_group(int S);
 int cm3p_attn_bwd_fused(const void* qkv, const void* out, const void* dout, const float* lse, void* dqkv, const uint8_t* key_mask,
```

Measured after the change: 196.9 pairs/s. Within noise of the previous version (-0.1%).
